# yewzijian/RegTR

Hardware: AMD Instinct MI355X
Metric: point-cloud pairs/sec (3DMatch ~20k pts) (higher is better)
Workload: dtype f32 (f16-pair split, 22-bit operands)

## Files before the change

### include/regtr_hip.h

```cpp
#ifndef REGTR_HIP_H
#define REGTR_HIP_H

#include <stddef.h>

#ifdef __cplusplus
extern "C" {
#endif

#define REGTR_OK 0
#define REGTR_ERR_LAUNCH (-1)
#define REGTR_ERR_ARG (-2)
#define REGTR_ERR_WORKSPACE (-3)

#define REGTR_ABI_VERSION 11
int regtr_abi_version(void);

#define REGTR_STATUS_F16_RANGE 1
#define REGTR_STATUS_NONFINITE_POSE 2


size_t regtr_grid_subsample_ws_bytes(int n_cap, int n_clouds);

int regtr_grid_subsample(const float* xyz, const int* seg_off, int n_clouds, int n_cap, float dl, float* out_xyz,
                         int* out_seg_off, void* ws, size_t ws_bytes, void* stream);

size_t regtr_grid_subsample_ordered_ws_bytes(int n_cap, int n_clouds, int row_order);
int regtr_grid_subsample_ordered(const float* xyz, const int* seg_off, int n_clouds, int n_cap, float dl, int row_order, int key_mode,
                                 int out_cap, float* out_xyz, int* out_seg_off, void* ws, size_t ws_bytes, void* stream);

size_t regtr_cellgrid_ws_bytes(int ns_cap, int n_clouds);

int regtr_cellgrid_build(const float* s_xyz, const int* s_seg_off, int n_clouds, int ns_cap, float radius, void* ws,
                         size_t ws_bytes, void* stream);

int regtr_radius_query(const float* q_xyz, const int* q_seg_off, int nq_cap, const int* s_seg_off, int ns_cap,
                       int n_clouds, float radius, int K, int order, const void* grid_ws, size_t ws_bytes, int* out_idx,
                       int* out_count, int* out_max_count, void* stream);

int regtr_radius_query_self(const int* s_seg_off, int ns_cap, int n_clouds, float radius, int K, int order, const void* grid_ws,
                            size_t ws_bytes, int* out_idx, int* out_count, int* out_max_count, void* stream);


int regtr_nearest_in_radius(const float* q_xyz, const int* q_seg_off, int nq_cap, const int* s_seg_off, int ns_cap,
                            int n_clouds, double radius, float grid_radius, const void* grid_ws, size_t ws_bytes, int* out_idx,
                            void* stream);

int regtr_overlap_avgpool(const float* ov, int ns, const int* nbr, int ld_nbr, int nq, int H, float* out, void* stream);



int regtr_rowsum_positive(const float* x, int n, int C, const float* stats, const int* seg_off, int n_seg, float slope,
                          float* flag, void* stream);

int regtr_kpconv_gather_computes_flag(int Cin, int H);

int regtr_kpconv_gather(const float* q_xyz, int nq, const float* s_xyz, int ns, const int* nbr, int H, const float* x,
                        int Cin, const float* flag, const float* s_xyzf, const float* kernel_points, int KP, float extent,
                        const float* x_stats, const int* q_seg_off, int n_seg, float slope, float* wf, int ld_wf, float* num,
                        void* stream);

int regtr_maxpool_gather(const float* x, int ns, int C, const int* nbr, int ld_nbr, int nq, int H, float* out, void* stream);

size_t regtr_instnorm_ws_bytes(int n_clouds, int max_len, int C);
int regtr_instnorm_stats(const float* x, const int* seg_off, int n_clouds, int max_len, int C, float eps, float* stats,
                         void* ws, size_t ws_bytes, void* stream);
int regtr_instnorm_apply(const float* x, const int* seg_off, int n_clouds, int max_len, int C, const float* stats,
                         const float* residual, const float* res_stats, int act, float slope, float* y, const float* row_xyz,
                         float* row_positive, void* stream);


size_t regtr_gemm_f32_ws_bytes(int M, int N, int K);
int regtr_gemm_f32(const float* A, int lda, const float* B, int ldb, float* C, int ldc, int M, int N, int K,
                   const float* bias, const float* row_div, const float* residual, int ldr, int act,
                   const float* a_stats, const int* a_seg_off, int n_seg, float a_slope, void* ws, size_t ws_bytes,
                   void* stream);

int regtr_gemm_x3_supported(int M, int N, int K);
int regtr_gemm_x3_preferred(int M, int N, int K);
size_t regtr_gemm_split_weights_bytes(int N, int K);
int regtr_gemm_split_weights(const float* W, int ld, int N, int K, int transposed, void* planes, void* stream);
int regtr_gemm_x3_f16_supported(int M, int N, int K, int with_stats);
size_t regtr_gemm_split_weights_f16_bytes(int N, int K);
int regtr_gemm_split_weights_f16(const float* W, int ld, int N, int K, int transposed, void* planes, void* stream);
size_t regtr_gemm_x3_ws_bytes(int M, int N, int K);
int regtr_gemm_x3(const float* A, int lda, const void* planes, float* C, int ldc, int M, int N, int K,
                  const float* bias, const float* row_div, const float* residual, int ldr, int act,
                  const float* a_stats, const int* a_seg_off, int n_seg, float a_slope, void* ws, size_t ws_bytes,
                  double* stat_partial, const int* stat_seg_off, int n_stat_seg, int n_planes, const void* tile_info, int* status,
                  void* stream);
int regtr_tile_segments(const int* seg_off, int n_seg, int M, int rows, void* out, void* stream);
int regtr_gemm_x3_tile_rows(int M, int N, int K);
int regtr_gemm_stream_supported(int M, int N, int K);
int regtr_gemm_stream_tile_rows(void);
int regtr_gemm_stream(const float* A, int lda, const void* planes, float* C, int ldc, int M, int N, int K,
                      const float* a_stats, float a_slope, const int* seg_off, int n_seg, const void* tile_info,
                      double* stat_partial, void* stream);
int regtr_block_tail_supported(int M, int N, int K1, int K2);
size_t regtr_block_tail_ws_bytes(int n_clouds, int max_len, int N, int K1, int K2);
int regtr_block_tail(const float* A1, int lda1, const float* a1_stats, float a1_slope, const float* row_div1, const float* A2, int lda2,
                     const float* W1, const float* W2, const int* seg_off, int n_clouds, int max_len, const void* tile_info,
                     int M, int N, int K1, int K2, float eps, float slope, float* Y, int ldy, void* ws, size_t ws_bytes,
                     float* out_stats, void* stream);

int regtr_gemm_x3_stat_tile_rows(int M, int N, int K);
int regtr_instnorm_finalize_tiles(const double* partial, const int* seg_off, int n_clouds, int C, int tile_rows, float eps,
                                  float* stats, void* stream);

int regtr_add_f32(const float* a, const float* b, size_t n, float* out, void* stream);

int regtr_layernorm(const float* x, int n, int D, const float* gamma, const float* beta, float eps, const float* add,
                    float* y, float* y_plain, void* stream);

int regtr_posemb_sine(const float* xyz, int n, int npf, int d_model, float scale, const float* dim_t, float* pe,
                      void* stream);


int regtr_mha_fwd(const float* q, int ldq, const float* k, int ldk, const float* v, int ldv, float* out, int ldo,
                  const int* seg_off, const int* kv_of, int n_clouds, int max_len, int n_heads, int head_dim, float scale,
                  int precision, int* status, void* stream);

int regtr_cross_encoder_per_layer_params(void);
int regtr_cross_encoder_supported(int n_tok, int d_model, int d_ff, int n_heads);
size_t regtr_cross_encoder_ws_bytes(int n_tok, int d_model, int d_ff);
int regtr_cross_encoder_fwd(const float* x, int n_tok, int d_model, int d_ff, int n_heads, int n_layers,
                            const void* const* layer_params, const float* layer_eps, const float* final_gamma,
                            const float* final_beta, float final_eps, int return_intermediate, const float* pe,
                            const int* seg_off, const int* kv_self, const int* kv_cross, int n_clouds, int max_len,
                            int gemm_planes, int attn_precision, void* ws, size_t ws_bytes, float* outs, int* status, void* stream);

typedef struct {
    const float* kn;
    const void* planes;
    const void* planes16;
    int N, K;
} regtr_weight_t;
typedef struct {
    int kind;
    int strided;
    int layer;
    int n_kp;
    float extent;
    const float* kernel_points;
    regtr_weight_t unary1;
    regtr_weight_t conv;
    regtr_weight_t unary2;
    regtr_weight_t shortcut;
} regtr_encoder_block_t;
typedef struct {
    const float* points;
    int n;
    const int* conv_idx;
    const int* pool_idx;
    int K;
    int pool_width;
    const int* seg_off;
    int max_len;
} regtr_encoder_level_t;
int regtr_encoder_supported(const regtr_encoder_block_t* blocks, int n_blocks, const regtr_encoder_level_t* levels, int n_levels,
                            int n_clouds, int first, int last);
size_t regtr_encoder_ws_bytes(const regtr_encoder_block_t* blocks, int n_blocks, const regtr_encoder_level_t* levels, int n_levels,
                              int n_clouds, int first, int last, int f16_pair);
int regtr_encoder_fwd(const regtr_encoder_block_t* blocks, int n_blocks, const regtr_encoder_level_t* levels, int n_levels, int n_clouds,
                      int first, int last, const float* x_in, float* out, int f16_pair, float slope, float eps, void* ws, size_t ws_bytes,
                      int* status, void* stream);

int regtr_attn_xyz(const float* q, const float* k, const float* xyz, float* out, const int* seg_off, const int* kv_of,
                   int n_clouds, int n_total, int n_layers, int max_len, int head_dim, float scale, void* stream);

int regtr_weighted_procrustes(const float* kp, const float* corr, const float* logit, const int* seg_off, int n_pairs,
                              int n_total, int n_layers, float* pose, int* status, void* stream);



size_t regtr_infonce_ws_bytes(int n_pairs, int max_anc);
int regtr_infonce(const float* anc, int ld_anc, const float* pos, int ld_pos, const float* anc_xyz, const float* pos_xyz,
                  const int* anc_seg_off, const int* pos_seg_off, int n_pairs, int n_anc, int n_pos, int max_anc, int D,
                  float r_p, float r_n, const float* anc_pose, float* pair_out, float* row_loss, float* row_mask, void* ws,
                  size_t ws_bytes, void* stream);

int regtr_se3_transform(const float* xyz, const int* seg_off, int n_clouds, int n, const float* pose, int pose_stride, float* out,
                        void* stream);

int regtr_loss_terms(const float* logit, const float* gt_overlap, const float* kp, const float* warped, const int* seg_off,
                     int n_pairs, int n_total, const float* pose, int pose_stride, float* out, void* stream);



int regtr_infonce_rows(const float* anc, int ld_anc, const float* pos, int ld_pos, const float* anc_xyz, const float* pos_xyz,
                       const int* anc_seg_off, const int* pos_seg_off, int n_pairs, int n_anc, int n_pos, int max_anc, int D,
                       float r_p, float r_n, const float* anc_pose, float* pair_out, float* row_loss, float* row_mask, float* row_lse,
                       int* row_idx, void* ws, size_t ws_bytes, void* stream);

int regtr_infonce_bwd(const float* anc, int ld_anc, const float* pos, int ld_pos, const float* anc_xyz, const float* pos_xyz,
                      const int* anc_seg_off, const int* pos_seg_off, int n_pairs, int n_anc, int n_pos, int max_anc, int max_pos,
                      int D, float r_n, const float* anc_pose, const float* row_lse, const int* row_idx, const float* row_mask,
                      const float* pair_out, const float* grad, float mean_div, float* d_anc, int ld_danc, float* d_pos, int ld_dpos,
                      void* stream);

size_t regtr_gemm_tn_ws_bytes(int M, int N1, int N2);
int regtr_gemm_tn(const float* a, int lda, const float* b, int ldb, int M, int N1, int N2, int fold, float* out, int ldo, void* ws,
                  size_t ws_bytes, void* stream);

int regtr_corr_l1_bwd(const float* kp, const float* warped, const float* w, const int* seg_off, int n_clouds, int n, const float* pose,
                      int pose_stride, const float* grad, const float* den, float* d_warped, void* stream);

size_t regtr_mha_bwd_ws_bytes(int n_total, int n_heads);
int regtr_mha_bwd(const float* q, int ldq, const float* k, int ldk, const float* v, int ldv, const float* d_out, int ld_do,
                  float* dq, int ld_dq, float* dk, int ld_dk, float* dv, int ld_dv, const int* seg_off, const int* kv_of,
                  int n_clouds, int n_total, int max_len, int n_heads, int head_dim, float scale, void* ws, size_t ws_bytes,
                  void* stream);

size_t regtr_layernorm_bwd_ws_bytes(int n, int D);
int regtr_layernorm_bwd(const float* x, int n, int D, const float* gamma, float eps, const float* dy, const float* dres, float* dx,
                        float* dgamma, float* dbeta, void* ws, size_t ws_bytes, void* stream);

size_t regtr_bias_relu_bwd_ws_bytes(int n, int N);
int regtr_bias_relu_bwd(const float* g, int ldg, const float* h, int ldh, float* dh, int ld_dh, float* db, int n, int N, void* ws,
                        size_t ws_bytes, void* stream);


size_t regtr_nbr_transpose_ws_bytes(int nq, int H, int ns);
int regtr_nbr_transpose(const int* nbr, int nq, int H, int ns, int* row_off, int* entries, void* ws, size_t ws_bytes, void* stream);

int regtr_kpconv_gather_bwd(const float* dwf, const float* q_xyz, int nq, const float* s_xyz, int ns, int H, int Cin,
                            const float* kernel_points, int KP, float extent, const int* row_off, const int* entries, float* dx,
                            void* stream);

int regtr_row_div(const float* x, int ldx, const float* div, int n, int N, float* out, int ldo, void* stream);

size_t regtr_gemm_tn_any_ws_bytes(int M, int N1, int N2);
int regtr_gemm_tn_any(const float* a, int lda, const float* b, int ldb, int M, int N1, int N2, float* out, int ldo, void* ws,
                      size_t ws_bytes, void* stream);

#ifdef __cplusplus
}
#endif
#endif
```

### regtr_amd/_lib.py

```python
import ctypes
import os
import threading

import torch

from . import context

_HERE = os.path.dirname(os.path.abspath(__file__))
LIB_PATH = os.path.join(_HERE, 'libregtr_hip.so')
if os.environ.get('REGTR_DEV', '') == '1' and os.environ.get('REGTR_VARIANT'):
    LIB_PATH = os.path.join(_HERE, f"libregtr_hip.{os.environ['REGTR_VARIANT']}.so")

_c = ctypes
_P = _c.c_void_p
_I = _c.c_int
_F = _c.c_float
_Z = _c.c_size_t

class Weight(_c.Structure):
    _fields_ = [('kn', _P), ('planes', _P), ('planes16', _P), ('N', _I), ('K', _I)]


class EncoderBlock(_c.Structure):
    _fields_ = [('kind', _I), ('strided', _I), ('layer', _I), ('n_kp', _I), ('extent', _F), ('kernel_points', _P),
                ('unary1', Weight), ('conv', Weight), ('unary2', Weight), ('shortcut', Weight)]


class EncoderLevel(_c.Structure):
    _fields_ = [('points', _P), ('n', _I), ('conv_idx', _P), ('pool_idx', _P), ('K', _I), ('pool_width', _I), ('seg_off', _P), ('max_len', _I)]


ABI_VERSION = 11

PARITY_SIGNATURES = {
    'regtr_parity_abi_version': (_I, []),
    'regtr_kdtree_ws_bytes': (_Z, [_I, _I]),
    'regtr_kdtree_query_scratch_bytes': (_Z, [_I]),
    'regtr_kdtree_build': (_I, [_P, _P, _I, _I, _P, _Z, _P]),
    'regtr_kdtree_radius_query': (_I, [_P, _P, _I, _P, _P, _I, _I, _F, _I, _I, _P, _Z, _P, _Z, _P, _P, _P, _P, _P]),
}

SIGNATURES = {
    'regtr_abi_version': (_I, []),
    'regtr_grid_subsample_ws_bytes': (_Z, [_I, _I]),
    'regtr_grid_subsample': (_I, [_P, _P, _I, _I, _F, _P, _P, _P, _Z, _P]),
    'regtr_grid_subsample_ordered_ws_bytes': (_Z, [_I, _I, _I]),
    'regtr_grid_subsample_ordered': (_I, [_P, _P, _I, _I, _F, _I, _I, _I, _P, _P, _P, _Z, _P]),
    'regtr_cellgrid_ws_bytes': (_Z, [_I, _I]),
    'regtr_cellgrid_build': (_I, [_P, _P, _I, _I, _F, _P, _Z, _P]),
    'regtr_radius_query': (_I, [_P, _P, _I, _P, _I, _I, _F, _I, _I, _P, _Z, _P, _P, _P, _P]),
    'regtr_radius_query_self': (_I, [_P, _I, _I, _F, _I, _I, _P, _Z, _P, _P, _P, _P]),
    'regtr_nearest_in_radius': (_I, [_P, _P, _I, _P, _I, _I, _c.c_double, _F, _P, _Z, _P, _P]),
    'regtr_overlap_avgpool': (_I, [_P, _I, _P, _I, _I, _I, _P, _P]),
    'regtr_rowsum_positive': (_I, [_P, _I, _I, _P, _P, _I, _F, _P, _P]),
    'regtr_kpconv_gather_computes_flag': (_I, [_I, _I]),
    'regtr_kpconv_gather': (_I, [_P, _I, _P, _I, _P, _I, _P, _I, _P, _P, _P, _I, _F, _P, _P, _I, _F, _P, _I, _P, _P]),
    'regtr_maxpool_gather': (_I, [_P, _I, _I, _P, _I, _I, _I, _P, _P]),
    'regtr_instnorm_ws_bytes': (_Z, [_I, _I, _I]),
    'regtr_instnorm_stats': (_I, [_P, _P, _I, _I, _I, _F, _P, _P, _Z, _P]),
    'regtr_instnorm_apply': (_I, [_P, _P, _I, _I, _I, _P, _P, _P, _I, _F, _P, _P, _P, _P]),
    'regtr_gemm_f32_ws_bytes': (_Z, [_I, _I, _I]),
    'regtr_gemm_f32': (_I, [_P, _I, _P, _I, _P, _I, _I, _I, _I, _P, _P, _P, _I, _I, _P, _P, _I, _F, _P, _Z, _P]),
    'regtr_gemm_x3_supported': (_I, [_I, _I, _I]),
    'regtr_gemm_x3_preferred': (_I, [_I, _I, _I]),
    'regtr_gemm_split_weights_bytes': (_Z, [_I, _I]),
    'regtr_gemm_split_weights': (_I, [_P, _I, _I, _I, _I, _P, _P]),
    'regtr_gemm_x3_f16_supported': (_I, [_I, _I, _I, _I]),
    'regtr_gemm_split_weights_f16_bytes': (_Z, [_I, _I]),
    'regtr_gemm_split_weights_f16': (_I, [_P, _I, _I, _I, _I, _P, _P]),
    'regtr_gemm_x3_ws_bytes': (_Z, [_I, _I, _I]),
    'regtr_gemm_x3': (_I, [_P, _I, _P, _P, _I, _I, _I, _I, _P, _P, _P, _I, _I, _P, _P, _I, _F, _P, _Z, _P, _P, _I, _I, _P, _P, _P]),
    'regtr_tile_segments': (_I, [_P, _I, _I, _I, _P, _P]),
    'regtr_gemm_x3_tile_rows': (_I, [_I, _I, _I]),
    'regtr_gemm_stream_supported': (_I, [_I, _I, _I]),
    'regtr_gemm_stream_tile_rows': (_I, []),
    'regtr_block_tail_supported': (_I, [_I, _I, _I, _I]),
    'regtr_block_tail_ws_bytes': (_Z, [_I, _I, _I, _I, _I]),
    'regtr_block_tail': (_I, [_P, _I, _P, _F, _P, _P, _I, _P, _P, _P, _I, _I, _P, _I, _I, _I, _I, _F, _F, _P, _I, _P, _Z, _P, _P]),
    'regtr_gemm_stream': (_I, [_P, _I, _P, _P, _I, _I, _I, _I, _P, _F, _P, _I, _P, _P, _P]),
    'regtr_gemm_x3_stat_tile_rows': (_I, [_I, _I, _I]),
    'regtr_instnorm_finalize_tiles': (_I, [_P, _P, _I, _I, _I, _F, _P, _P]),
    'regtr_add_f32': (_I, [_P, _P, _Z, _P, _P]),
    'regtr_layernorm': (_I, [_P, _I, _I, _P, _P, _F, _P, _P, _P, _P]),
    'regtr_posemb_sine': (_I, [_P, _I, _I, _I, _F, _P, _P, _P]),
    'regtr_mha_fwd': (_I, [_P, _I, _P, _I, _P, _I, _P, _I, _P, _P, _I, _I, _I, _I, _F, _I, _P, _P]),
    'regtr_cross_encoder_per_layer_params': (_I, []),
    'regtr_cross_encoder_supported': (_I, [_I, _I, _I, _I]),
    'regtr_cross_encoder_ws_bytes': (_Z, [_I, _I, _I]),
    'regtr_cross_encoder_fwd': (_I, [_P, _I, _I, _I, _I, _I, _P, _P, _P, _P, _F, _I, _P, _P, _P, _P, _I, _I, _I, _I, _P, _Z, _P, _P, _P]),
    'regtr_encoder_supported': (_I, [_P, _I, _P, _I, _I, _I, _I]),
    'regtr_encoder_ws_bytes': (_Z, [_P, _I, _P, _I, _I, _I, _I, _I]),
    'regtr_encoder_fwd': (_I, [_P, _I, _P, _I, _I, _I, _I, _P, _P, _I, _F, _F, _P, _Z, _P, _P]),
    'regtr_attn_xyz': (_I, [_P, _P, _P, _P, _P, _P, _I, _I, _I, _I, _I, _F, _P]),
    'regtr_weighted_procrustes': (_I, [_P, _P, _P, _P, _I, _I, _I, _P, _P, _P]),
    'regtr_infonce_ws_bytes': (_Z, [_I, _I]),
    'regtr_infonce': (_I, [_P, _I, _P, _I, _P, _P, _P, _P, _I, _I, _I, _I, _I, _F, _F, _P, _P, _P, _P, _P, _Z, _P]),
    'regtr_loss_terms': (_I, [_P, _P, _P, _P, _P, _I, _I, _P, _I, _P, _P]),
    'regtr_se3_transform': (_I, [_P, _P, _I, _I, _P, _I, _P, _P]),
    'regtr_infonce_rows': (_I, [_P, _I, _P, _I, _P, _P, _P, _P, _I, _I, _I, _I, _I, _F, _F, _P, _P, _P, _P, _P, _P, _P, _Z, _P]),
    'regtr_infonce_bwd': (_I, [_P, _I, _P, _I, _P, _P, _P, _P, _I, _I, _I, _I, _I, _I, _F, _P, _P, _P, _P, _P, _P, _F, _P, _I, _P, _I,
                               _P]),
    'regtr_gemm_tn_ws_bytes': (_Z, [_I, _I, _I]),
    'regtr_gemm_tn': (_I, [_P, _I, _P, _I, _I, _I, _I, _I, _P, _I, _P, _Z, _P]),
    'regtr_corr_l1_bwd': (_I, [_P, _P, _P, _P, _I, _I, _P, _I, _P, _P, _P, _P]),
    'regtr_mha_bwd_ws_bytes': (_Z, [_I, _I]),
    'regtr_mha_bwd': (_I, [_P, _I, _P, _I, _P, _I, _P, _I, _P, _I, _P, _I, _P, _I, _P, _P, _I, _I, _I, _I, _I, _F, _P, _Z, _P]),
    'regtr_layernorm_bwd_ws_bytes': (_Z, [_I, _I]),
    'regtr_layernorm_bwd': (_I, [_P, _I, _I, _P, _F, _P, _P, _P, _P, _P, _P, _Z, _P]),
    'regtr_bias_relu_bwd_ws_bytes': (_Z, [_I, _I]),
    'regtr_bias_relu_bwd': (_I, [_P, _I, _P, _I, _P, _I, _P, _I, _I, _P, _Z, _P]),
    'regtr_nbr_transpose_ws_bytes': (_Z, [_I, _I, _I]),
    'regtr_nbr_transpose': (_I, [_P, _I, _I, _I, _P, _P, _P, _Z, _P]),
    'regtr_kpconv_gather_bwd': (_I, [_P, _P, _I, _P, _I, _I, _I, _P, _I, _F, _P, _P, _P, _P]),
    'regtr_row_div': (_I, [_P, _I, _P, _I, _I, _P, _I, _P]),
    'regtr_gemm_tn_any_ws_bytes': (_Z, [_I, _I, _I]),
    'regtr_gemm_tn_any': (_I, [_P, _I, _P, _I, _I, _I, _I, _P, _I, _P, _Z, _P]),
}

COMPOSITE = ('regtr_encoder_fwd', 'regtr_cross_encoder_fwd')

_ERR = {-1: 'kernel launch failed', -2: 'invalid argument', -3: 'workspace too small'}

_lib = None
_load_lock = threading.Lock()


def lib():
    global _lib
    if _lib is None:
        with _load_lock:
            if _lib is None:
                _lib = _load()
    return _lib


def _load():
    _lib = None
    if True:
        if not os.path.exists(LIB_PATH):
            raise RuntimeError(f'{LIB_PATH} is missing: build it with `python -m regtr_amd.build` '
                               '(hipcc --offload-arch=gfx950). There is no CPU fallback.')
        _lib = ctypes.PyDLL(LIB_PATH)
        for name, (res, args) in SIGNATURES.items():
            fn = getattr(_lib, name)
            fn.restype = res
            fn.argtypes = args
        nogil = ctypes.CDLL(LIB_PATH)
        for name in COMPOSITE:
            fn = getattr(nogil, name)
            fn.restype, fn.argtypes = SIGNATURES[name]
            setattr(_lib, name, fn)
        got = _lib.regtr_abi_version()
        if got != ABI_VERSION:
            _lib = None
            raise RuntimeError(f'{LIB_PATH} implements C-ABI version {got}, this binding was written for {ABI_VERSION}: rebuild with '
                               '`python -m regtr_amd.build --force`')
    return _lib


_parity = None
PARITY_LIB_PATH = os.path.join(_HERE, 'libregtr_parity.so')


def parity_lib():
    global _parity
    if _parity is None:
        with _load_lock:
            if _parity is None:
                if not os.path.exists(PARITY_LIB_PATH):
                    raise RuntimeError(f'{PARITY_LIB_PATH} is missing: build it with `python -m regtr_amd.build` (parity mode only)')
                lib_ = ctypes.PyDLL(PARITY_LIB_PATH)
                for name, (res, args) in PARITY_SIGNATURES.items():
                    fn = getattr(lib_, name)
                    fn.restype, fn.argtypes = res, args
                if lib_.regtr_parity_abi_version() != ABI_VERSION:
                    raise RuntimeError(f'{PARITY_LIB_PATH} was built against C-ABI version {lib_.regtr_parity_abi_version()}, this binding is {ABI_VERSION}: '
                                       'rebuild with `python -m regtr_amd.build --force`')
                _parity = lib_
    return _parity


def check(status, what):
    if status != 0:
        raise RuntimeError(f'{what}: {_ERR.get(status, "error")} (status {status})')


on_device = context.on_device


def ptr(t, dtype=torch.float32):
    if t is None:
        return None
    dev = context.current().device_index
    if t.get_device() != (dev if dev is not None else torch.cuda.current_device()) or t.dtype is not dtype or not t.is_contiguous():
        _explain(t, dtype)
    return t.data_ptr()


def _explain(t, dtype):
    if not t.is_cuda:
        raise RuntimeError('regtr_amd ops need GPU tensors (no CPU fallback)')
    if t.dtype != dtype:
        raise RuntimeError(f'regtr_amd op expected a {dtype} tensor, got {t.dtype} (the kernels reinterpret nothing)')
    if not t.is_contiguous():
        raise RuntimeError('regtr_amd ops need contiguous tensors')
    dev = context.current().device_index
    raise RuntimeError(f'tensor on {t.device} but the launch device is cuda:{dev if dev is not None else torch.cuda.current_device()}; '
                       'wrap the call in regtr_amd._lib.on_device(tensor.device)')


def iptr(t):
    return ptr(t, torch.int32)


def bptr(t):
    return ptr(t, torch.uint8)


def dptr(t):
    return ptr(t, torch.float64)


def raw(t):
    if t is None:
        return None
    if t.dtype is not torch.float32 or t.get_device() < 0:
        raise RuntimeError(f'regtr_amd op expected a float32 GPU tensor, got {t.dtype} on {t.device}')
    return t.data_ptr()


_raw_stream = getattr(torch._C, '_cuda_getCurrentRawStream', None)


def stream():
    dev = context.current().device_index
    if _raw_stream is not None:
        return _raw_stream(dev if dev is not None else torch.cuda.current_device())
    return torch.cuda.current_stream().cuda_stream
```

### regtr_amd/csrc/attention.hip

```cpp
#include "common.h"
#include "mfma_operands.h"

namespace {

constexpr int HD = 32;
constexpr int TQ = 32, TK = 32;
constexpr int LDS_STRIDE = HD + 1;

struct MhaArgs {
    const float* q; const float* k; const float* v;
    float* out;
    const int* seg_off; const int* kv_of;
    int ldq, ldk, ldv, ldo, n_heads;
    float scale;
    int* status;
};

__device__ __forceinline__ int acc_row(int r, int hi) { return (r & 3) + 8 * (r >> 2) + 4 * hi; }

template <int KS>
__global__ void __launch_bounds__(KS * RG_WAVE) __attribute__((amdgpu_waves_per_eu(2))) k_mha_fwd(MhaArgs g)
{
    __shared__ float KVs[KS][2 * TK * LDS_STRIDE];
    const int lane = threadIdx.x & 63, l31 = lane & 31, hi = lane >> 5;
    const int wave = __builtin_amdgcn_readfirstlane(threadIdx.x >> 6);
    float* Ks = KVs[wave];
    float* Vs = KVs[wave] + TK * LDS_STRIDE;
    const int cloud = blockIdx.z, head = blockIdx.y;
    const int q_begin = g.seg_off[cloud], q_end = g.seg_off[cloud + 1];
    const int q0 = q_begin + blockIdx.x * TQ;
    if (q0 >= q_end) return;
    const int kc = g.kv_of[cloud];
    const int k_begin = g.seg_off[kc], nk = g.seg_off[kc + 1] - k_begin;
    const int hoff = head * HD;

    float qreg[16];
    {
        const int qrow = q0 + l31;
        const bool live = qrow < q_end;
        const float* qp = g.q + (size_t)(live ? qrow : q_begin) * g.ldq + hoff + hi;
        const float scl = live ? g.scale : 0.f;
#pragma unroll
        for (int s = 0; s < 16; s++) qreg[s] = qp[2 * s] * scl;
    }

    floatx16 o;
#pragma unroll
    for (int r = 0; r < 16; r++) o[r] = 0.f;
    float m_run = -INFINITY, l_run = 0.f;

    float4 kreg[4], vreg[4];
    auto fetch = [&](int kt) {
#pragma unroll
        for (int it = 0; it < 4; it++) {
            const int krow = min(kt + it * 8 + (lane >> 3), nk > 0 ? nk - 1 : 0), c4 = (lane & 7) * 4;
            const int kb = nk > 0 ? k_begin : q_begin;
            kreg[it] = *(const float4*)(g.k + (size_t)(kb + krow) * g.ldk + hoff + c4);
            vreg[it] = *(const float4*)(g.v + (size_t)(kb + krow) * g.ldv + hoff + c4);
        }
    };
    fetch(wave * TK);
    for (int kt = wave * TK; kt < nk; kt += KS * TK) {
        __builtin_amdgcn_wave_barrier();
#pragma unroll
        for (int it = 0; it < 4; it++) {
            const int row = it * 8 + (lane >> 3), c4 = (lane & 7) * 4;
            float* kd = &Ks[row * LDS_STRIDE + c4];
            kd[0] = kreg[it].x; kd[1] = kreg[it].y; kd[2] = kreg[it].z; kd[3] = kreg[it].w;
            float* vd = &Vs[row * LDS_STRIDE + c4];
            vd[0] = vreg[it].x; vd[1] = vreg[it].y; vd[2] = vreg[it].z; vd[3] = vreg[it].w;
        }
        __builtin_amdgcn_wave_barrier();
        fetch(kt + KS * TK);

        floatx16 sc;
#pragma unroll
        for (int r = 0; r < 16; r++) sc[r] = 0.f;
#pragma unroll
        for (int s = 0; s < 16; s++)
            sc = __builtin_amdgcn_mfma_f32_32x32x2f32(Ks[l31 * LDS_STRIDE + 2 * s + hi], qreg[s], sc, 0, 0, 0);

        float mx = -INFINITY;
#pragma unroll
        for (int r = 0; r < 16; r++) {
            if (kt + acc_row(r, hi) >= nk) sc[r] = -INFINITY;
            mx = fmaxf(mx, sc[r]);
        }
        mx = fmaxf(mx, __shfl_xor(mx, 32, RG_WAVE));
        const float m_new = fmaxf(m_run, mx);
        const float alpha = expf(m_run - m_new);
        float psum = 0.f;
#pragma unroll
        for (int r = 0; r < 16; r++) {
            sc[r] = expf(sc[r] - m_new);
            psum += sc[r];
        }
        psum += __shfl_xor(psum, 32, RG_WAVE);
        l_run = l_run * alpha + psum;
        m_run = m_new;
#pragma unroll
        for (int r = 0; r < 16; r++) o[r] *= alpha;

#pragma unroll
        for (int s = 0; s < 16; s++)
            o = __builtin_amdgcn_mfma_f32_32x32x2f32(Vs[acc_row(s, hi) * LDS_STRIDE + l31], sc[s], o, 0, 0, 0);
    }

    if (KS > 1) {
        __builtin_amdgcn_wave_barrier();
        float* mine = KVs[wave];
        if (wave > 0) {
#pragma unroll
            for (int r = 0; r < 16; r++) mine[r * 64 + lane] = o[r];
            mine[16 * 64 + lane] = m_run;
            mine[17 * 64 + lane] = l_run;
        }
        __syncthreads();
        if (wave > 0) return;
#pragma unroll 1
        for (int w = 1; w < KS; w++) {
            const float* p = KVs[w];
            const float mw = p[16 * 64 + lane], lw = p[17 * 64 + lane];
            if (mw == -INFINITY) continue;
            const float m_new = fmaxf(m_run, mw);
            const float a0 = expf(m_run - m_new), a1 = expf(mw - m_new);
            l_run = l_run * a0 + lw * a1;
#pragma unroll
            for (int r = 0; r < 16; r++) o[r] = o[r] * a0 + p[r * 64 + lane] * a1;
            m_run = m_new;
        }
    }

    const int qrow = q0 + l31;
    if (qrow < q_end) {
        const float inv = l_run > 0.f ? 1.0f / l_run : 0.f;
        float* dst = g.out + (size_t)qrow * g.ldo + hoff;
#pragma unroll
        for (int r4 = 0; r4 < 4; r4++) {
            const int d = 8 * r4 + 4 * hi;
            *(float4*)(dst + d) = make_float4(o[4 * r4] * inv, o[4 * r4 + 1] * inv, o[4 * r4 + 2] * inv, o[4 * r4 + 3] * inv);
        }
    }
}

constexpr int BW = 4;
constexpr int BW8 = 8;
constexpr int BROW = 64;

#ifndef MHA_WAVES_ATTR
#define MHA_WAVES_ATTR __attribute__((amdgpu_waves_per_eu(3)))
#endif
#ifndef MHA_WIDE_MIN_WG
#define MHA_WIDE_MIN_WG 4096
#endif
template <int NP, bool F16 = false>
__device__ __forceinline__ void bf_split8(const float (&x)[8], bf16x8 (&f)[NP])
{
    unsigned w[4][NP];
#pragma unroll
    for (int i = 0; i < 4; i++) rg_split2<NP, F16>(x[2 * i], x[2 * i + 1], w[i]);
#pragma unroll
    for (int p = 0; p < NP; p++) f[p] = __builtin_bit_cast(bf16x8, make_uint4(w[0][p], w[1][p], w[2][p], w[3][p]));
}
template <int NP>
__device__ __forceinline__ floatx16 bf_mma(const bf16x8 (&a)[NP], const bf16x8 (&b)[NP], floatx16 c)
{
    if (NP == 3) {
        c = __builtin_amdgcn_mfma_f32_32x32x16_bf16(a[2], b[0], c, 0, 0, 0);
        c = __builtin_amdgcn_mfma_f32_32x32x16_bf16(a[1], b[1], c, 0, 0, 0);
        c = __builtin_amdgcn_mfma_f32_32x32x16_bf16(a[0], b[2], c, 0, 0, 0);
    }
    if (NP >= 2) {
        c = __builtin_amdgcn_mfma_f32_32x32x16_bf16(a[1], b[0], c, 0, 0, 0);
        c = __builtin_amdgcn_mfma_f32_32x32x16_bf16(a[0], b[1], c, 0, 0, 0);
    }
    return __builtin_amdgcn_mfma_f32_32x32x16_bf16(a[0], b[0], c, 0, 0, 0);
}

__device__ __forceinline__ void f16_mma(const bf16x8 (&a)[2], const bf16x8 (&b)[2], floatx16& hi, floatx16& lo)
{
    lo = __builtin_amdgcn_mfma_f32_32x32x16_f16(__builtin_bit_cast(f16x8, a[1]), __builtin_bit_cast(f16x8, b[0]), lo, 0, 0, 0);
    hi = __builtin_amdgcn_mfma_f32_32x32x16_f16(__builtin_bit_cast(f16x8, a[0]), __builtin_bit_cast(f16x8, b[0]), hi, 0, 0, 0);
    lo = __builtin_amdgcn_mfma_f32_32x32x16_f16(__builtin_bit_cast(f16x8, a[0]), __builtin_bit_cast(f16x8, b[1]), lo, 0, 0, 0);
}

__device__ __forceinline__ float mha_max_halves(float x)
{
    const auto r = __builtin_amdgcn_permlane32_swap(__float_as_uint(x), __float_as_uint(x), false, false);
    return fmaxf(__uint_as_float(r[0]), __uint_as_float(r[1]));
}
__device__ __forceinline__ float mha_sum_halves(float x)
{
    const auto r = __builtin_amdgcn_permlane32_swap(__float_as_uint(x), __float_as_uint(x), false, false);
    return __uint_as_float(r[0]) + __uint_as_float(r[1]);
}

template <int NP, bool F16 = false, int NW = BW>
__global__ void __launch_bounds__(NW * RG_WAVE) MHA_WAVES_ATTR k_mha_fwd_bf16(MhaArgs g)
{
    __shared__ __align__(16) unsigned char Ks[2][NP][TK * BROW];
    __shared__ __align__(16) unsigned char Vt[2][NP][HD * BROW];
    const int t = threadIdx.x, lane = t & 63, l31 = lane & 31, hi = lane >> 5;
    const int wave = __builtin_amdgcn_readfirstlane(t >> 6);
    const int cloud = blockIdx.z, head = blockIdx.y;
    const int q_begin = g.seg_off[cloud], q_end = g.seg_off[cloud + 1];
    if (q_begin + (int)blockIdx.x * NW * TQ >= q_end) return;
    const int q0 = q_begin + (blockIdx.x * NW + wave) * TQ;
    const bool wave_live = q0 < q_end;
    const int kc = g.kv_of[cloud];
    const int k_begin = g.seg_off[kc], nk = g.seg_off[kc + 1] - k_begin;
    const int hoff = head * HD;

    bf16x8 qf[2][NP];
    {
        const int qrow = q0 + l31;
        const bool live = wave_live && qrow < q_end;
        const float sc2 = g.scale * 1.44269504088896340736f;
        const float* qp = g.q + (size_t)(live ? qrow : q_begin) * g.ldq + hoff + 8 * hi;
        float4 qv[2][2];
#pragma unroll
        for (int ks = 0; ks < 2; ks++) { qv[ks][0] = *(const float4*)(qp + 16 * ks); qv[ks][1] = *(const float4*)(qp + 16 * ks + 4); }
        const float scl = live ? sc2 : 0.f;
#pragma unroll
        for (int ks = 0; ks < 2; ks++) {
            const float x[8] = {qv[ks][0].x * scl, qv[ks][0].y * scl, qv[ks][0].z * scl, qv[ks][0].w * scl,
                                qv[ks][1].x * scl, qv[ks][1].y * scl, qv[ks][1].z * scl, qv[ks][1].w * scl};
            bf_split8<NP, F16>(x, qf[ks]);
        }
    }

    constexpr int KPT = NW == 4 ? 4 : 2;
    const int skey = t / (32 / KPT), sdk = (t % (32 / KPT)) * KPT;
    const int su = NW == 4 ? t >> 4 : t >> 5, sd2 = NW == 4 ? (t & 15) * 2 : (t & 31);
    const unsigned k_dst = (unsigned)skey * BROW + (((unsigned)(sdk >> 3) ^ (((unsigned)skey >> 2) & 3u)) * 16u) + ((unsigned)sdk & 7u) * 2u;
    const unsigned vpos = ((2u * su) & 0x13u) | (((2u * su) & 4u) << 1) | (((2u * su) & 8u) >> 1);
    unsigned v_dst[2];
#pragma unroll
    for (int dd = 0; dd < 2; dd++) {
        const unsigned row = (unsigned)(sd2 + dd);
        v_dst[dd] = row * BROW + (((vpos >> 3) ^ ((row >> 2) & 3u)) * 16u) + (vpos & 7u) * 2u;
    }
    struct KV { float4 k; float2 v0, v1; };
    const int nk1 = nk > 0 ? nk - 1 : 0;
    const int kb = nk > 0 ? k_begin : q_begin;
    auto fetch = [&](KV& r, int kt) {
        const int kr = min(kt + skey, nk1), v0 = min(kt + 2 * su, nk1), v1 = min(kt + 2 * su + 1, nk1);
        if constexpr (NW == 4) {
            r.k = *(const float4*)(g.k + (size_t)(kb + kr) * g.ldk + hoff + sdk);
            r.v0 = *(const float2*)(g.v + (size_t)(kb + v0) * g.ldv + hoff + sd2);
            r.v1 = *(const float2*)(g.v + (size_t)(kb + v1) * g.ldv + hoff + sd2);
        } else {
            const float2 k2 = *(const float2*)(g.k + (size_t)(kb + kr) * g.ldk + hoff + sdk);
            r.k.x = k2.x; r.k.y = k2.y;
            r.v0.x = g.v[(size_t)(kb + v0) * g.ldv + hoff + sd2];
            r.v1.x = g.v[(size_t)(kb + v1) * g.ldv + hoff + sd2];
        }
    };
    auto stage = [&](const KV& r, int buf) {
        unsigned a[NP], b[NP];
        rg_split2<NP, F16>(r.k.x, r.k.y, a);
        if constexpr (NW == 4) {
            rg_split2<NP, F16>(r.k.z, r.k.w, b);
#pragma unroll
            for (int p = 0; p < NP; p++) *(uint2*)(&Ks[buf][p][k_dst]) = make_uint2(a[p], b[p]);
        } else {
#pragma unroll
            for (int p = 0; p < NP; p++) *(unsigned*)(&Ks[buf][p][k_dst]) = a[p];
        }
        rg_split2<NP, F16>(r.v0.x, r.v1.x, a);
        if constexpr (NW == 4) rg_split2<NP, F16>(r.v0.y, r.v1.y, b);
#pragma unroll
        for (int p = 0; p < NP; p++) {
            *(unsigned*)(&Vt[buf][p][v_dst[0]]) = a[p];
            if constexpr (NW == 4) *(unsigned*)(&Vt[buf][p][v_dst[1]]) = b[p];
        }
    };

    floatx16 o, o_lo;
#pragma unroll
    for (int r = 0; r < 16; r++) { o[r] = 0.f; o_lo[r] = 0.f; }
    float m_run = -INFINITY, l_run = 0.f;
    unsigned f_off[2];
#pragma unroll
    for (int ks = 0; ks < 2; ks++) f_off[ks] = (unsigned)l31 * BROW + ((((unsigned)(2 * ks + hi)) ^ (((unsigned)l31 >> 2) & 3u)) * 16u);

#ifdef MHA_PROF
    long long pt[6] = {0, 0, 0, 0, 0, 0}, pc = clock64(), pstart = pc;
#define MHA_STAMP(I) do { const long long n_ = clock64(); pt[I] += n_ - pc; pc = n_; } while (0)
#else
#define MHA_STAMP(I) do {} while (0)
#endif
    KV ra, rb;
    fetch(ra, 0);
    stage(ra, 0);
    fetch(ra, TK);
    __syncthreads();
    MHA_STAMP(0);
    auto tile = [&](int kt, int buf, KV& rold, KV& rnew) {
        const bool more = kt + TK < nk;
        fetch(rnew, kt + 2 * TK);
        MHA_STAMP(1);
        if (wave_live) {
            floatx16 sc, sc_lo;
#pragma unroll
            for (int r = 0; r < 16; r++) { sc[r] = 0.f; sc_lo[r] = 0.f; }
#pragma unroll
            for (int ks = 0; ks < 2; ks++) {
                bf16x8 kf[NP];
#pragma unroll
                for (int p = 0; p < NP; p++) kf[p] = __builtin_bit_cast(bf16x8, *(const uint4*)(&Ks[buf][p][f_off[ks]]));
                if constexpr (F16) f16_mma(kf, qf[ks], sc, sc_lo);
                else sc = bf_mma<NP>(kf, qf[ks], sc);
            }
            if constexpr (F16) {
                rg_fold_low(sc, sc_lo);
            }
            MHA_STAMP(2);
            if (kt + TK > nk) {
#pragma unroll
                for (int r = 0; r < 16; r++)
                    if (kt + acc_row(r, hi) >= nk) sc[r] = -INFINITY;
            }
            float mx = -INFINITY;
#pragma unroll
            for (int r = 0; r < 16; r++) mx = fmaxf(mx, sc[r]);
            mx = mha_max_halves(mx);
            const float m_new = fmaxf(m_run, mx);
            const float alpha = __builtin_amdgcn_exp2f(m_run - m_new);
            float pr[16];
            float psum = 0.f;
#pragma unroll
            for (int r = 0; r < 16; r++) { pr[r] = __builtin_amdgcn_exp2f(sc[r] - m_new); psum += pr[r]; }
            psum = mha_sum_halves(psum);
            l_run = l_run * alpha + psum;
            m_run = m_new;
#pragma unroll
            for (int r = 0; r < 16; r++) { o[r] *= alpha; if (F16) o_lo[r] *= alpha; }
#pragma unroll
            for (int ks = 0; ks < 2; ks++) {
                float x[8];
#pragma unroll
                for (int j = 0; j < 8; j++) x[j] = pr[8 * ks + j];
                bf16x8 pf[NP], vf[NP];
                bf_split8<NP, F16>(x, pf);
#pragma unroll
                for (int p = 0; p < NP; p++) vf[p] = __builtin_bit_cast(bf16x8, *(const uint4*)(&Vt[buf][p][f_off[ks]]));
                if constexpr (F16) f16_mma(vf, pf, o, o_lo);
                else o = bf_mma<NP>(vf, pf, o);
            }
            MHA_STAMP(3);
        }
        if (more) stage(rold, buf ^ 1);
        MHA_STAMP(4);
        __syncthreads();
        MHA_STAMP(5);
    };
    for (int kt = 0; kt < nk; kt += 2 * TK) {
        tile(kt, 0, ra, rb);
        if (kt + TK >= nk) break;
        tile(kt + TK, 1, rb, ra);
    }
#ifdef MHA_PROF
    if ((blockIdx.z == 3 || blockIdx.z == 77) && blockIdx.y == 2 && lane == 0)
        printf("mha NP %d cloud %d wg %d wave %d live %d nk %d: prologue %lld fetch-issue %lld qk %lld softmax+pv %lld stage %lld barrier %lld total %lld (cycles)\n", NP,
               (int)blockIdx.z, (int)blockIdx.x, wave, (int)wave_live, nk, pt[0], pt[1], pt[2], pt[3], pt[4], pt[5], clock64() - pstart);
#endif

    if constexpr (F16) {
        const float chk = fmaf(l_run, 0.f, rg_fold_low(o, o_lo));
        rg_report_range(g.status, chk, wave_live);
    }
    const int qrow = q0 + l31;
    if (wave_live && qrow < q_end) {
        const float inv = l_run > 0.f ? 1.0f / l_run : 0.f;
        float* dst = g.out + (size_t)qrow * g.ldo + hoff;
#pragma unroll
        for (int r4 = 0; r4 < 4; r4++) {
            const int d = 8 * r4 + 4 * hi;
            *(float4*)(dst + d) = make_float4(o[4 * r4] * inv, o[4 * r4 + 1] * inv, o[4 * r4 + 2] * inv, o[4 * r4 + 3] * inv);
        }
    }
}

struct AttnXyzArgs {
    const float* q; const float* k; const float* xyz; float* out;
    const int* seg_off; const int* kv_of;
    int n_total;
    float scale;
};

template <int HDX>
__global__ void __launch_bounds__(RG_WAVE) __attribute__((amdgpu_waves_per_eu(2))) k_attn_xyz(AttnXyzArgs g)
{
    constexpr int KS = HDX + 1;
    extern __shared__ float smem_x[];
    float* Ks = smem_x;
    float* Vs = smem_x + TK * KS;
    const int lane = threadIdx.x, l31 = lane & 31, hi = lane >> 5;
    const int cloud = blockIdx.z, layer = blockIdx.y;
    const int q_begin = g.seg_off[cloud], q_end = g.seg_off[cloud + 1];
    const int q0 = q_begin + blockIdx.x * TQ;
    if (q0 >= q_end) return;
    const int kc = g.kv_of[cloud];
    const int k_begin = g.seg_off[kc], nk = g.seg_off[kc + 1] - k_begin;
    const float* Q = g.q + (size_t)layer * g.n_total * HDX;
    const float* K = g.k + (size_t)layer * g.n_total * HDX;

    float qreg[HDX / 2];
    {
        const int qrow = q0 + l31;
        const bool live = qrow < q_end;
        const float* qp = Q + (size_t)(live ? qrow : q_begin) * HDX + hi;
        const float scl = live ? g.scale : 0.f;
#pragma unroll
        for (int s = 0; s < HDX / 2; s++) qreg[s] = qp[2 * s] * scl;
    }
    floatx16 o;
#pragma unroll
    for (int r = 0; r < 16; r++) o[r] = 0.f;
    float m_run = -INFINITY, l_run = 0.f;
    for (int e = lane; e < TK * LDS_STRIDE; e += RG_WAVE) Vs[e] = 0.f;

    constexpr int LPR = HDX / 4 < RG_WAVE ? HDX / 4 : RG_WAVE;
    const int c4 = (lane < LPR ? lane : LPR - 1) * 4;
    const int nk1 = nk > 0 ? nk - 1 : 0;
    const int kb = nk > 0 ? k_begin : q_begin;
    for (int kt = 0; kt < nk; kt += TK) {
        __syncthreads();
#pragma unroll 1
        for (int row0 = 0; row0 < TK; row0 += 8) {
            float4 v[8];
#pragma unroll
            for (int i = 0; i < 8; i++) v[i] = *(const float4*)(K + (size_t)(kb + min(kt + row0 + i, nk1)) * HDX + c4);
            if (lane < LPR) {
#pragma unroll
                for (int i = 0; i < 8; i++) {
                    float* kd = &Ks[(row0 + i) * KS + c4];
                    kd[0] = v[i].x; kd[1] = v[i].y; kd[2] = v[i].z; kd[3] = v[i].w;
                }
            }
        }
        {
            const float* xp = g.xyz + (size_t)(kb + min(kt + l31, nk1)) * 3;
            const float x = xp[0], y = xp[1], z = xp[2];
            if (hi == 0) { Vs[l31 * LDS_STRIDE] = x; Vs[l31 * LDS_STRIDE + 1] = y; Vs[l31 * LDS_STRIDE + 2] = z; }
        }
        __syncthreads();

        floatx16 sc;
#pragma unroll
        for (int r = 0; r < 16; r++) sc[r] = 0.f;
#pragma unroll
        for (int s = 0; s < HDX / 2; s++)
            sc = __builtin_amdgcn_mfma_f32_32x32x2f32(Ks[l31 * KS + 2 * s + hi], qreg[s], sc, 0, 0, 0);

        float mx = -INFINITY;
#pragma unroll
        for (int r = 0; r < 16; r++) {
            if (kt + acc_row(r, hi) >= nk) sc[r] = -INFINITY;
            mx = fmaxf(mx, sc[r]);
        }
        mx = fmaxf(mx, __shfl_xor(mx, 32, RG_WAVE));
        const float m_new = fmaxf(m_run, mx);
        const float alpha = expf(m_run - m_new);
        float psum = 0.f;
#pragma unroll
        for (int r = 0; r < 16; r++) {
            sc[r] = expf(sc[r] - m_new);
            psum += sc[r];
        }
        psum += __shfl_xor(psum, 32, RG_WAVE);
        l_run = l_run * alpha + psum;
        m_run = m_new;
#pragma unroll
        for (int r = 0; r < 16; r++) o[r] *= alpha;
#pragma unroll
        for (int s = 0; s < 16; s++)
            o = __builtin_amdgcn_mfma_f32_32x32x2f32(Vs[acc_row(s, hi) * LDS_STRIDE + l31], sc[s], o, 0, 0, 0);
    }
    const int qrow = q0 + l31;
    if (qrow < q_end && hi == 0) {
        const float inv = l_run > 0.f ? 1.0f / l_run : 0.f;
        float* dst = g.out + ((size_t)layer * g.n_total + qrow) * 3;
        dst[0] = o[0] * inv; dst[1] = o[1] * inv; dst[2] = o[2] * inv;
    }
}

}

extern "C" {

int regtr_mha_fwd(const float* q, int ldq, const float* k, int ldk, const float* v, int ldv, float* out, int ldo,
                  const int* seg_off, const int* kv_of, int n_clouds, int max_len, int n_heads, int head_dim, float scale,
                  int precision, int* status, void* stream)
{
    if (!q || !k || !v || !out || !seg_off || !kv_of || n_clouds < 1 || n_heads < 1 || max_len < 0) return RG_ERR_ARG;
    if (head_dim != HD || precision < 0 || precision > 3) return RG_ERR_ARG;
    if ((ldq | ldk | ldv | ldo) % 4 || (((uintptr_t)q | (uintptr_t)k | (uintptr_t)v | (uintptr_t)out) % 16)) return RG_ERR_ARG;
    if (max_len == 0) return RG_OK;
    MhaArgs g{q, k, v, out, seg_off, kv_of, ldq, ldk, ldv, ldo, n_heads, scale, status};
    hipStream_t st = (hipStream_t)stream;
    const bool small = (long long)rg_cdiv(max_len, BW * TQ) * n_heads * n_clouds < 512;
    if (precision == 2 || ((precision == 0 || precision == 3) && small)) {
        const dim3 grid(rg_cdiv(max_len, TQ), n_heads, n_clouds);
        if ((long long)grid.x * grid.y * grid.z <= 1024 && max_len > 4 * TK) k_mha_fwd<4><<<grid, 4 * RG_WAVE, 0, st>>>(g);
        else k_mha_fwd<1><<<grid, RG_WAVE, 0, st>>>(g);
    }
    else {
        if ((ldv % 2) || ((uintptr_t)v % 8)) return RG_ERR_ARG;
        if (max_len > BW * TQ && (long long)rg_cdiv(max_len, BW8 * TQ) * n_heads * n_clouds >= MHA_WIDE_MIN_WG) {
            const dim3 grid(rg_cdiv(max_len, BW8 * TQ), n_heads, n_clouds);
            if (precision == 0) k_mha_fwd_bf16<3, false, BW8><<<grid, BW8 * RG_WAVE, 0, st>>>(g);
            else if (precision == 3) k_mha_fwd_bf16<2, true, BW8><<<grid, BW8 * RG_WAVE, 0, st>>>(g);
            else k_mha_fwd_bf16<1, false, BW8><<<grid, BW8 * RG_WAVE, 0, st>>>(g);
        } else {
            const dim3 grid(rg_cdiv(max_len, BW * TQ), n_heads, n_clouds);
            if (precision == 0) k_mha_fwd_bf16<3><<<grid, BW * RG_WAVE, 0, st>>>(g);
            else if (precision == 3) k_mha_fwd_bf16<2, true><<<grid, BW * RG_WAVE, 0, st>>>(g);
            else k_mha_fwd_bf16<1><<<grid, BW * RG_WAVE, 0, st>>>(g);
        }
    }
    RG_RETURN_IF_LAUNCH_FAILED();
    return RG_OK;
}

int regtr_attn_xyz(const float* q, const float* k, const float* xyz, float* out, const int* seg_off, const int* kv_of,
                   int n_clouds, int n_total, int n_layers, int max_len, int head_dim, float scale, void* stream)
{
    if (!q || !k || !xyz || !out || !seg_off || !kv_of || n_clouds < 1 || n_total < 0 || n_layers < 1 || max_len < 0)
        return RG_ERR_ARG;
    if ((((uintptr_t)q | (uintptr_t)k) % 16)) return RG_ERR_ARG;
    if (max_len == 0 || n_total == 0) return RG_OK;
    AttnXyzArgs g{q, k, xyz, out, seg_off, kv_of, n_total, scale};
    const dim3 grid(rg_cdiv(max_len, TQ), n_layers, n_clouds);
    hipStream_t st = (hipStream_t)stream;
#define RG_ATTN_XYZ(HDX_) k_attn_xyz<HDX_><<<grid, RG_WAVE, (TK * (HDX_ + 1) + TK * LDS_STRIDE) * sizeof(float), st>>>(g)
    if (head_dim == 256) RG_ATTN_XYZ(256);
    else if (head_dim == 128) RG_ATTN_XYZ(128);
    else if (head_dim == 64) RG_ATTN_XYZ(64);
    else if (head_dim == 32) RG_ATTN_XYZ(32);
    else return RG_ERR_ARG;
#undef RG_ATTN_XYZ
    RG_RETURN_IF_LAUNCH_FAILED();
    return RG_OK;
}

}
```

### regtr_amd/csrc/cross_encoder.hip

```cpp
#include <math.h>

#include "common.h"

namespace {

enum {
    CE_N1_G, CE_N1_B, CE_SA_IN_W, CE_SA_IN_B, CE_SA_OUT_W, CE_SA_OUT_B,
    CE_N2_G, CE_N2_B, CE_CA_IN_W, CE_CA_IN_B, CE_CA_OUT_W, CE_CA_OUT_B,
    CE_N3_G, CE_N3_B, CE_L1_W, CE_L1_B, CE_L2_W, CE_L2_B, CE_PER_LAYER
};

size_t ce_gemm_ws(int M, int D, int F)
{
    size_t w = regtr_gemm_x3_ws_bytes(M, 3 * D, D);
    const size_t a = regtr_gemm_x3_ws_bytes(M, D, D), b = regtr_gemm_x3_ws_bytes(M, F, D), c = regtr_gemm_x3_ws_bytes(M, D, F);
    if (a > w) w = a;
    if (b > w) w = b;
    if (c > w) w = c;
    return w;
}

}

extern "C" {

int regtr_cross_encoder_per_layer_params(void) { return CE_PER_LAYER; }

int regtr_cross_encoder_supported(int n_tok, int d_model, int d_ff, int n_heads)
{
    if (n_tok < 1 || d_model < 64 || d_ff < 64 || n_heads < 1 || d_model % n_heads || d_model / n_heads != 32) return 0;
    return (regtr_gemm_x3_preferred(n_tok, 3 * d_model, d_model) && regtr_gemm_x3_preferred(n_tok, d_model, d_model) &&
            regtr_gemm_x3_preferred(n_tok, d_ff, d_model) && regtr_gemm_x3_preferred(n_tok, d_model, d_ff)) ? 1 : 0;
}

size_t regtr_cross_encoder_ws_bytes(int n_tok, int d_model, int d_ff)
{
    const size_t row = (size_t)n_tok * sizeof(float);
    return 6 * 256 + row * ((size_t)d_model * 4 + 3 * (size_t)d_model + d_ff) + rg_align_up(ce_gemm_ws(n_tok, d_model, d_ff), 256) + 256;
}

int regtr_cross_encoder_fwd(const float* x, int n_tok, int d_model, int d_ff, int n_heads, int n_layers,
                            const void* const* layer_params, const float* layer_eps, const float* final_gamma,
                            const float* final_beta, float final_eps, int return_intermediate, const float* pe,
                            const int* seg_off, const int* kv_self, const int* kv_cross, int n_clouds, int max_len,
                            int gemm_planes, int attn_precision, void* ws, size_t ws_bytes, float* outs, int* status, void* stream)
{
    if (!x || !layer_params || !layer_eps || !seg_off || !kv_self || !kv_cross || !outs || n_layers < 1 || n_clouds < 1) return RG_ERR_ARG;
    if (!regtr_cross_encoder_supported(n_tok, d_model, d_ff, n_heads)) return RG_ERR_ARG;
    if (!ws || ws_bytes < regtr_cross_encoder_ws_bytes(n_tok, d_model, d_ff)) return RG_ERR_WORKSPACE;
    const int M = n_tok, D = d_model, F = d_ff, hd = D / n_heads;
    RgCarver cv(ws, ws_bytes);
    float* x2p = cv.take<float>((size_t)M * D);
    float* qkv = cv.take<float>((size_t)M * 3 * D);
    float* att = cv.take<float>((size_t)M * D);
    float* xa = cv.take<float>((size_t)M * D);
    float* xb = cv.take<float>((size_t)M * D);
    float* h = cv.take<float>((size_t)M * F);
    const size_t gws_bytes = ce_gemm_ws(M, D, F);
    void* gws = gws_bytes ? (void*)cv.take<char>(gws_bytes) : nullptr;
    if (!cv.ok()) return RG_ERR_WORKSPACE;
    const float scale = (float)(1.0 / sqrt((double)hd));

#define CE_TRY(call) do { const int st_ = (call); if (st_ != RG_OK) return st_; } while (0)
    auto gemm = [&](const float* A, int K, const void* W, const void* bias, float* C, int N, const float* residual, int relu) {
        return regtr_gemm_x3(A, K, W, C, N, M, N, K, (const float*)bias, nullptr, residual, residual ? D : 0, relu, nullptr, nullptr, 0,
                             0.1f, gws, gws_bytes, nullptr, nullptr, 0, gemm_planes, nullptr, status, stream);
    };
    auto attention = [&](const float* xin, const void* const* P, int g, int in_w, float eps, const int* kv_of, float* xout) {
        int st = regtr_layernorm(xin, M, D, (const float*)P[g], (const float*)P[g + 1], eps, pe, x2p, nullptr, stream);
        if (st != RG_OK) return st;
        st = gemm(x2p, D, P[in_w], P[in_w + 1], qkv, 3 * D, nullptr, 0);
        if (st != RG_OK) return st;
        st = regtr_mha_fwd(qkv, 3 * D, qkv + D, 3 * D, qkv + 2 * D, 3 * D, att, D, seg_off, kv_of, n_clouds, max_len, n_heads, hd, scale,
                           attn_precision, status, stream);
        if (st != RG_OK) return st;
        return gemm(att, D, P[in_w + 2], P[in_w + 3], xout, D, xin, 0);
    };

    const float* cur = x;
    for (int l = 0; l < n_layers; l++) {
        const void* const* P = layer_params + (size_t)l * CE_PER_LAYER;
        const float* eps = layer_eps + 3 * l;
        float* t1 = (cur == xa) ? xb : xa;
        float* t2 = (t1 == xa) ? xb : xa;
        CE_TRY(attention(cur, P, CE_N1_G, CE_SA_IN_W, eps[0], kv_self, t1));
        CE_TRY(attention(t1, P, CE_N2_G, CE_CA_IN_W, eps[1], kv_cross, t2));
        CE_TRY(regtr_layernorm(t2, M, D, (const float*)P[CE_N3_G], (const float*)P[CE_N3_B], eps[2], nullptr, x2p, nullptr, stream));
        CE_TRY(gemm(x2p, D, P[CE_L1_W], P[CE_L1_B], h, F, nullptr, 1));
        CE_TRY(gemm(h, F, P[CE_L2_W], P[CE_L2_B], t1, D, t2, 0));
        cur = t1;
        if (return_intermediate || l == n_layers - 1) {
            float* o = outs + (return_intermediate ? (size_t)l * M * D : 0);
            if (final_gamma) CE_TRY(regtr_layernorm(cur, M, D, final_gamma, final_beta, final_eps, nullptr, o, nullptr, stream));
            else if (hipMemcpyAsync(o, cur, (size_t)M * D * sizeof(float), hipMemcpyDeviceToDevice, (hipStream_t)stream) != hipSuccess)
                return RG_ERR_LAUNCH;
        }
    }
#undef CE_TRY
    return RG_OK;
}

}
```

### regtr_amd/csrc/norm.hip

```cpp
#include "common.h"

namespace {

constexpr int IN_ROWS = 128;

inline int in_rows(int max_len, int n_clouds, int C)
{
    const int TR = 256 / (C >> 2);
    int rows = IN_ROWS;
    while (rows > 4 * TR && rows > 8 && (long long)rg_cdiv(max_len > 0 ? max_len : 1, rows) * n_clouds < 1024) rows >>= 1;
    return rows;
}


__global__ void __launch_bounds__(256) k_instnorm_partial(const float* __restrict__ x, const int* __restrict__ seg_off, int C,
                                                          int nchunk, int rows, double2* __restrict__ partial)
{
    __shared__ double sh[256 * 8];
    const int b = blockIdx.y, chunk = blockIdx.x;
    const int r0 = seg_off[b] + chunk * rows, r1 = min(seg_off[b + 1], r0 + rows);
    if (r0 >= r1) return;
    const int C4 = C >> 2, TR = 256 / C4;
    const int tx = threadIdx.x % C4, ty = threadIdx.x / C4;
    double s[4] = {0, 0, 0, 0}, ss[4] = {0, 0, 0, 0};
    const float* base = x + 4 * tx;
    auto add = [&](const float4& v) {
        s[0] += v.x; s[1] += v.y; s[2] += v.z; s[3] += v.w;
        ss[0] += (double)v.x * v.x; ss[1] += (double)v.y * v.y; ss[2] += (double)v.z * v.z; ss[3] += (double)v.w * v.w;
    };
    int r = r0 + ty;
    for (; r + 3 * TR < r1; r += 4 * TR) {
        float4 v[4];
#pragma unroll
        for (int u = 0; u < 4; u++) v[u] = *(const float4*)(base + (size_t)(r + u * TR) * C);
#pragma unroll
        for (int u = 0; u < 4; u++) add(v[u]);
    }
    for (; r < r1; r += TR) add(*(const float4*)(base + (size_t)r * C));
#pragma unroll
    for (int j = 0; j < 4; j++) { sh[threadIdx.x * 8 + j] = s[j]; sh[threadIdx.x * 8 + 4 + j] = ss[j]; }
    __syncthreads();
    if (ty == 0) {
        for (int y = 1; y < TR; y++)
#pragma unroll
            for (int j = 0; j < 4; j++) { s[j] += sh[(y * C4 + tx) * 8 + j]; ss[j] += sh[(y * C4 + tx) * 8 + 4 + j]; }
        double2* o = partial + ((size_t)b * nchunk + chunk) * C + 4 * tx;
#pragma unroll
        for (int j = 0; j < 4; j++) o[j] = make_double2(s[j], ss[j]);
    }
}

__global__ void __launch_bounds__(256) k_instnorm_finalize(const double2* __restrict__ partial, const int* __restrict__ seg_off,
                                                           int C, int nchunk, int rows, float eps, float2* __restrict__ stats)
{
    const int b = blockIdx.y, c = blockIdx.x * (blockDim.x >> 6) + (threadIdx.x >> 6);
    if (c >= C) return;
    const int lane = rg_lane();
    const int n = seg_off[b + 1] - seg_off[b];
    const int used = (n + rows - 1) / rows;
    double s = 0, ss = 0;
    for (int k = lane; k < used; k += RG_WAVE) {
        const double2 p = partial[((size_t)b * nchunk + k) * C + c];
        s += p.x; ss += p.y;
    }
    s = rg_wave_sum(s); ss = rg_wave_sum(ss);
    if (lane == 0) {
        float mean = 0.f, rstd = 0.f;
        if (n > 0) {
            const double m = s / n;
            double var = ss / n - m * m;
            if (var < 0) var = 0;
            mean = (float)m;
            rstd = (float)(1.0 / sqrt(var + (double)eps));
        }
        stats[(size_t)b * C + c] = make_float2(mean, rstd);
    }
}

__global__ void __launch_bounds__(256) k_instnorm_finalize_tiles(const double2* __restrict__ partial, const int* __restrict__ seg_off,
                                                                 int C, int tile_rows, float eps, float2* __restrict__ stats)
{
    const int b = blockIdx.y, c = blockIdx.x * blockDim.x + threadIdx.x;
    if (c >= C) return;
    const int r0 = seg_off[b], r1 = seg_off[b + 1], n = r1 - r0;
    float mean = 0.f, rstd = 0.f;
    if (n > 0) {
        const int t0 = r0 / tile_rows, t1 = (r1 - 1) / tile_rows;
        const double2* p = partial + (size_t)(t0 + b) * C + c;
        double s = 0, ss = 0;
        int t = t0;
        for (; t + 3 <= t1; t += 4) {
            const double2 a0 = p[0], a1 = p[(size_t)C], a2 = p[2 * (size_t)C], a3 = p[3 * (size_t)C];
            s = (((s + a0.x) + a1.x) + a2.x) + a3.x; ss = (((ss + a0.y) + a1.y) + a2.y) + a3.y;
            p += 4 * (size_t)C;
        }
        for (; t <= t1; t++) { const double2 a = *p; s += a.x; ss += a.y; p += C; }
        const double m = s / n;
        double var = ss / n - m * m;
        if (var < 0) var = 0;
        mean = (float)m;
        rstd = (float)(1.0 / sqrt(var + (double)eps));
    }
    stats[(size_t)b * C + c] = make_float2(mean, rstd);
}

__global__ void __launch_bounds__(256) k_instnorm_finalize_tiles_wave(const double2* __restrict__ partial, const int* __restrict__ seg_off,
                                                                      int C, int tile_rows, float eps, float2* __restrict__ stats)
{
    const int b = blockIdx.y, c = blockIdx.x * (blockDim.x >> 6) + (threadIdx.x >> 6);
    if (c >= C) return;
    const int lane = rg_lane();
    const int r0 = seg_off[b], r1 = seg_off[b + 1], n = r1 - r0;
    float mean = 0.f, rstd = 0.f;
    if (n > 0) {
        const int t0 = r0 / tile_rows, t1 = (r1 - 1) / tile_rows;
        double s = 0, ss = 0;
        for (int t = t0 + lane; t <= t1; t += RG_WAVE) {
            const double2 a = partial[(size_t)(t + b) * C + c];
            s += a.x; ss += a.y;
        }
        s = rg_wave_sum(s); ss = rg_wave_sum(ss);
        const double m = s / n;
        double var = ss / n - m * m;
        if (var < 0) var = 0;
        mean = (float)m;
        rstd = (float)(1.0 / sqrt(var + (double)eps));
    }
    if (lane == 0) stats[(size_t)b * C + c] = make_float2(mean, rstd);
}

__global__ void __launch_bounds__(256) k_instnorm_apply(const float* __restrict__ x, const int* __restrict__ seg_off, int C,
                                                        const float2* __restrict__ stats, const float* __restrict__ res,
                                                        const float2* __restrict__ res_stats, int act, float slope,
                                                        float* __restrict__ y, const float* __restrict__ row_xyz,
                                                        float* __restrict__ row_positive, int rows)
{
    const int b = blockIdx.y, chunk = blockIdx.x;
    const int r0 = seg_off[b] + chunk * rows, r1 = min(seg_off[b + 1], r0 + rows);
    if (r0 >= r1) return;
    const int C4 = C >> 2, TR = 256 / C4;
    const int tx = threadIdx.x % C4, ty = threadIdx.x / C4;
    float mu[4] = {0.f, 0.f, 0.f, 0.f}, rs[4] = {1.f, 1.f, 1.f, 1.f}, rmu[4] = {0.f, 0.f, 0.f, 0.f}, rrs[4] = {1.f, 1.f, 1.f, 1.f};
    if (stats) {
        const float4* st = (const float4*)(stats + (size_t)b * C + 4 * tx);
        const float4 a = st[0], c = st[1];
        mu[0] = a.x; rs[0] = a.y; mu[1] = a.z; rs[1] = a.w; mu[2] = c.x; rs[2] = c.y; mu[3] = c.z; rs[3] = c.w;
    }
    if (res_stats) {
        const float4* st = (const float4*)(res_stats + (size_t)b * C + 4 * tx);
        const float4 a = st[0], c = st[1];
        rmu[0] = a.x; rrs[0] = a.y; rmu[1] = a.z; rrs[1] = a.w; rmu[2] = c.x; rrs[2] = c.y; rmu[3] = c.z; rrs[3] = c.w;
    }
    for (int r = r0 + ty; r < r1; r += 4 * TR) {
        float4 v[4], rv[4];
#pragma unroll
        for (int u = 0; u < 4; u++) v[u] = *(const float4*)(x + (size_t)min(r + u * TR, r1 - 1) * C + 4 * tx);
        if (res) {
#pragma unroll
            for (int u = 0; u < 4; u++) rv[u] = *(const float4*)(res + (size_t)min(r + u * TR, r1 - 1) * C + 4 * tx);
        }
#pragma unroll
        for (int u = 0; u < 4; u++) {
            const int rr = r + u * TR;
            if (rr >= r1) continue;
            float o[4] = {v[u].x, v[u].y, v[u].z, v[u].w};
#pragma unroll
            for (int j = 0; j < 4; j++) o[j] = (o[j] - mu[j]) * rs[j];
            if (res) {
                const float q[4] = {rv[u].x, rv[u].y, rv[u].z, rv[u].w};
#pragma unroll
                for (int j = 0; j < 4; j++) o[j] += (q[j] - rmu[j]) * rrs[j];
            }
            if (act == 1) {
#pragma unroll
                for (int j = 0; j < 4; j++) o[j] = o[j] > 0.f ? o[j] : o[j] * slope;
            }
            *(float4*)(y + (size_t)rr * C + 4 * tx) = make_float4(o[0], o[1], o[2], o[3]);
            if (row_positive) {
                float sum = (o[0] + o[1]) + (o[2] + o[3]);
                for (int m = 1; m < C4; m <<= 1) sum += __shfl_xor(sum, m, RG_WAVE);
                if (tx == 0) {
                    const float f = sum > 0.f ? 1.f : 0.f;
                    if (row_xyz) *(float4*)(row_positive + 4 * (size_t)rr) = make_float4(row_xyz[3 * (size_t)rr], row_xyz[3 * (size_t)rr + 1],
                                                                                         row_xyz[3 * (size_t)rr + 2], f);
                    else row_positive[rr] = f;
                }
            }
        }
    }
}

__global__ void __launch_bounds__(256) k_layernorm(const float* __restrict__ x, int n, int D, const float* __restrict__ gamma,
                                                   const float* __restrict__ beta, float eps, const float* __restrict__ add,
                                                   float* __restrict__ y, float* __restrict__ y_plain)
{
    const int row = blockIdx.x * (blockDim.x >> 6) + (threadIdx.x >> 6);
    if (row >= n) return;
    const int lane = rg_lane();
    const float* xr = x + (size_t)row * D;
    float s = 0.f;
    for (int c = lane * 4; c < D; c += RG_WAVE * 4) {
        const float4 v = *(const float4*)(xr + c);
        s += (v.x + v.y) + (v.z + v.w);
    }
    const float mean = rg_wave_sum(s) / (float)D;
    float ss = 0.f;
    for (int c = lane * 4; c < D; c += RG_WAVE * 4) {
        const float4 v = *(const float4*)(xr + c);
        const float a = v.x - mean, b = v.y - mean, cc = v.z - mean, d = v.w - mean;
        ss += (a * a + b * b) + (cc * cc + d * d);
    }
    const float rstd = 1.0f / sqrtf(rg_wave_sum(ss) / (float)D + eps);
    for (int c = lane * 4; c < D; c += RG_WAVE * 4) {
        const float4 v = *(const float4*)(xr + c);
        const float4 gm = *(const float4*)(gamma + c), bt = *(const float4*)(beta + c);
        float4 o = make_float4((v.x - mean) * rstd * gm.x + bt.x, (v.y - mean) * rstd * gm.y + bt.y,
                               (v.z - mean) * rstd * gm.z + bt.z, (v.w - mean) * rstd * gm.w + bt.w);
        if (y_plain) *(float4*)(y_plain + (size_t)row * D + c) = o;
        if (add) {
            const float4 a = *(const float4*)(add + (size_t)row * D + c);
            o.x += a.x; o.y += a.y; o.z += a.z; o.w += a.w;
        }
        *(float4*)(y + (size_t)row * D + c) = o;
    }
}

__global__ void __launch_bounds__(256) k_posemb_sine(const float* __restrict__ xyz, int n, int npf, int d_model, float scale,
                                                     const float* __restrict__ dim_t, float* __restrict__ pe)
{
    const size_t e = (size_t)blockIdx.x * blockDim.x + threadIdx.x;
    if (e >= (size_t)n * d_model) return;
    const int i = (int)(e / d_model), d = (int)(e % d_model);
    float v = 0.f;
    if (d < 3 * npf) {
        const int a = d / npf, f = d % npf;
        const float p = __fdiv_rn(__fmul_rn(xyz[3 * (size_t)i + a], scale), dim_t[f]);
        v = (f & 1) ? cosf(p) : sinf(p);
    }
    pe[e] = v;
}

}

extern "C" {

size_t regtr_instnorm_ws_bytes(int n_clouds, int max_len, int C)
{
    if (n_clouds < 1 || C < 4 || C % 4 || C > 1024 || 256 % (C / 4)) return 256;
    const size_t nchunk = (size_t)rg_cdiv(max_len > 0 ? max_len : 1, in_rows(max_len, n_clouds, C));
    return nchunk * n_clouds * C * sizeof(double2) + 256;
}

int regtr_instnorm_stats(const float* x, const int* seg_off, int n_clouds, int max_len, int C, float eps, float* stats,
                         void* ws, size_t ws_bytes, void* stream)
{
    if (!x || !seg_off || !stats || n_clouds < 1 || C < 4 || C % 4 || max_len < 0) return RG_ERR_ARG;
    if (C > 1024 || 256 % (C / 4)) return RG_ERR_ARG;
    if (ws_bytes < regtr_instnorm_ws_bytes(n_clouds, max_len, C)) return RG_ERR_WORKSPACE;
    if (max_len == 0) return RG_OK;
    hipStream_t st = (hipStream_t)stream;
    const int rows = in_rows(max_len, n_clouds, C);
    const int nchunk = rg_cdiv(max_len, rows);
    k_instnorm_partial<<<dim3(nchunk, n_clouds), 256, 0, st>>>(x, seg_off, C, nchunk, rows, (double2*)ws);
    k_instnorm_finalize<<<dim3(rg_cdiv(C, 4), n_clouds), 256, 0, st>>>((const double2*)ws, seg_off, C, nchunk, rows, eps,
                                                                         (float2*)stats);
    RG_RETURN_IF_LAUNCH_FAILED();
    return RG_OK;
}

int regtr_instnorm_finalize_tiles(const double* partial, const int* seg_off, int n_clouds, int C, int tile_rows, float eps,
                                  float* stats, void* stream)
{
    if (!partial || !seg_off || !stats || n_clouds < 1 || C < 1 || tile_rows < 1) return RG_ERR_ARG;
    if ((long long)n_clouds * C <= 4096) {
        k_instnorm_finalize_tiles_wave<<<dim3(rg_cdiv(C, 4), n_clouds), 256, 0, (hipStream_t)stream>>>(
            (const double2*)partial, seg_off, C, tile_rows, eps, (float2*)stats);
    } else {
        const int bs = C >= 256 ? 256 : (C >= 128 ? 128 : 64);
        k_instnorm_finalize_tiles<<<dim3(rg_cdiv(C, bs), n_clouds), bs, 0, (hipStream_t)stream>>>(
            (const double2*)partial, seg_off, C, tile_rows, eps, (float2*)stats);
    }
    RG_RETURN_IF_LAUNCH_FAILED();
    return RG_OK;
}

int regtr_instnorm_apply(const float* x, const int* seg_off, int n_clouds, int max_len, int C, const float* stats,
                         const float* residual, const float* res_stats, int act, float slope, float* y, const float* row_xyz,
                         float* row_positive, void* stream)
{
    if (!x || !seg_off || !y || n_clouds < 1 || C < 4 || C % 4 || max_len < 0) return RG_ERR_ARG;
    if (C > 1024 || 256 % (C / 4) || (row_positive && C > 256) || (row_xyz && (!row_positive || (uintptr_t)row_positive % 16)))
        return RG_ERR_ARG;
    if (max_len == 0) return RG_OK;
    const int rows = in_rows(max_len, n_clouds, C);
    k_instnorm_apply<<<dim3(rg_cdiv(max_len, rows), n_clouds), 256, 0, (hipStream_t)stream>>>(
        x, seg_off, C, (const float2*)stats, residual, (const float2*)res_stats, act, slope, y, row_xyz, row_positive, rows);
    RG_RETURN_IF_LAUNCH_FAILED();
    return RG_OK;
}

static __global__ void __launch_bounds__(256) k_add(const float* __restrict__ a, const float* __restrict__ b, size_t n, float* __restrict__ out)
{
    const size_t i = ((size_t)blockIdx.x * blockDim.x + threadIdx.x) * 4;
    if (i + 3 < n) {
        const float4 x = *(const float4*)(a + i), y = *(const float4*)(b + i);
        *(float4*)(out + i) = make_float4(x.x + y.x, x.y + y.y, x.z + y.z, x.w + y.w);
    } else {
        for (size_t j = i; j < n; j++) out[j] = a[j] + b[j];
    }
}

int regtr_add_f32(const float* a, const float* b, size_t n, float* out, void* stream)
{
    if (!a || !b || !out || (((uintptr_t)a | (uintptr_t)b | (uintptr_t)out) % 16)) return RG_ERR_ARG;
    if (n == 0) return RG_OK;
    k_add<<<rg_cdiv((long long)((n + 3) / 4), 256), 256, 0, (hipStream_t)stream>>>(a, b, n, out);
    RG_RETURN_IF_LAUNCH_FAILED();
    return RG_OK;
}

int regtr_layernorm(const float* x, int n, int D, const float* gamma, const float* beta, float eps, const float* add,
                    float* y, float* y_plain, void* stream)
{
    if (!x || !gamma || !beta || !y || n < 0 || D < 4 || D % 4) return RG_ERR_ARG;
    if (n == 0) return RG_OK;
    k_layernorm<<<rg_cdiv(n, 4), 256, 0, (hipStream_t)stream>>>(x, n, D, gamma, beta, eps, add, y, y_plain);
    RG_RETURN_IF_LAUNCH_FAILED();
    return RG_OK;
}

int regtr_posemb_sine(const float* xyz, int n, int npf, int d_model, float scale, const float* dim_t, float* pe,
                      void* stream)
{
    if (!xyz || !dim_t || !pe || n < 0 || npf < 1 || d_model < 3 * npf) return RG_ERR_ARG;
    if (n == 0) return RG_OK;
    k_posemb_sine<<<rg_cdiv((long long)n * d_model, 256), 256, 0, (hipStream_t)stream>>>(xyz, n, npf, d_model, scale,
                                                                                          dim_t, pe);
    RG_RETURN_IF_LAUNCH_FAILED();
    return RG_OK;
}

}
```

### regtr_amd/ops.py

```python
import math

import torch

from . import _lib, context
from ._lib import bptr, check, dptr, iptr, ptr, raw, stream


def _ws(nbytes, device):
    return torch.empty(int(nbytes), dtype=torch.uint8, device=device)


F16_OPERAND_LIMIT = 65504.0 / 2


VOXEL_KEY_MODES = {'origin': 0, 'floor': 1, 'floor_rcp': 2}


def grid_subsample(xyz, seg_off, n_cap, dl, row_order=0, key_mode=0, out_cap=None):
    L = _lib.lib()
    n_clouds = seg_off.numel() - 1
    out_cap = int(n_cap if out_cap is None else min(out_cap, n_cap))
    out = torch.empty((max(out_cap, 1), 3), dtype=torch.float32, device=xyz.device)
    out_off = torch.empty(n_clouds + 1, dtype=torch.int32, device=xyz.device)
    nb = L.regtr_grid_subsample_ordered_ws_bytes(n_cap, n_clouds, int(row_order))
    ws = _ws(nb, xyz.device)
    check(L.regtr_grid_subsample_ordered(ptr(xyz), iptr(seg_off), n_clouds, n_cap, float(dl), int(row_order), int(key_mode), out_cap, ptr(out),
                                         iptr(out_off), bptr(ws), nb, stream()), 'regtr_grid_subsample_ordered')
    return out, out_off


self_query_kernel = True
SELF_QUERY_MIN_POINTS = 262144


class CellGrid:

    def __init__(self, s_xyz, s_seg_off, ns_cap, radius):
        L = _lib.lib()
        self.n_clouds = s_seg_off.numel() - 1
        self.s_xyz, self.s_seg_off, self.ns_cap, self.radius = s_xyz, s_seg_off, int(ns_cap), float(radius)
        self.nbytes = L.regtr_cellgrid_ws_bytes(self.ns_cap, self.n_clouds)
        self.ws = _ws(self.nbytes, s_xyz.device)
        check(L.regtr_cellgrid_build(ptr(s_xyz), iptr(s_seg_off), self.n_clouds, self.ns_cap, self.radius, bptr(self.ws),
                                     self.nbytes, stream()), 'regtr_cellgrid_build')

    def query(self, q_xyz, q_seg_off, nq_cap, K, want_count=False, order=0):
        L = _lib.lib()
        idx = torch.empty((max(nq_cap, 1), K), dtype=torch.int32, device=q_xyz.device)
        cnt = mx = None
        if want_count:
            cnt = torch.empty(max(nq_cap, 1), dtype=torch.int32, device=q_xyz.device)
            mx = torch.zeros(1, dtype=torch.int32, device=q_xyz.device)
        if self_query_kernel and q_xyz is self.s_xyz and q_seg_off is self.s_seg_off and self.ns_cap >= SELF_QUERY_MIN_POINTS:
            check(L.regtr_radius_query_self(iptr(self.s_seg_off), self.ns_cap, self.n_clouds, self.radius, int(K), int(order),
                                            bptr(self.ws), self.nbytes, iptr(idx), iptr(cnt), iptr(mx), stream()), 'regtr_radius_query_self')
        else:
            check(L.regtr_radius_query(ptr(q_xyz), iptr(q_seg_off), int(nq_cap), iptr(self.s_seg_off), self.ns_cap,
                                       self.n_clouds, self.radius, int(K), int(order), bptr(self.ws), self.nbytes, iptr(idx), iptr(cnt),
                                       iptr(mx), stream()), 'regtr_radius_query')
        return (idx, cnt, mx) if want_count else idx


class KdTree:

    def __init__(self, s_xyz, s_seg_off, ns_cap):
        L = _lib.parity_lib()
        self.n_clouds = s_seg_off.numel() - 1
        self.s_xyz, self.s_seg_off, self.ns_cap = s_xyz, s_seg_off, int(ns_cap)
        self.nbytes = L.regtr_kdtree_ws_bytes(self.ns_cap, self.n_clouds)
        self.ws = _ws(self.nbytes, s_xyz.device)
        check(L.regtr_kdtree_build(ptr(s_xyz), iptr(s_seg_off), self.n_clouds, self.ns_cap, bptr(self.ws), self.nbytes, stream()),
              'regtr_kdtree_build')

    def query(self, q_xyz, q_seg_off, nq_cap, radius, K, list_cap=128):
        L = _lib.parity_lib()
        dev = q_xyz.device
        idx = torch.empty((max(nq_cap, 1), K), dtype=torch.int32, device=dev)
        while True:
            st = torch.zeros(2, dtype=torch.int32, device=dev)
            sb = L.regtr_kdtree_query_scratch_bytes(int(list_cap))
            scratch = _ws(sb, dev)
            check(L.regtr_kdtree_radius_query(ptr(q_xyz), iptr(q_seg_off), int(nq_cap), ptr(self.s_xyz), iptr(self.s_seg_off),
                                              self.ns_cap, self.n_clouds, float(radius), int(K), int(list_cap), bptr(self.ws),
                                              self.nbytes, bptr(scratch), sb, iptr(idx), None, st.data_ptr(), st.data_ptr() + 4,
                                              stream()), 'regtr_kdtree_radius_query')
            max_count, overflow = (int(v) for v in st.cpu())
            if overflow:
                raise RuntimeError('regtr_kdtree_radius_query: traversal stack overflow (tree deeper than the parity mode supports)')
            if max_count <= list_cap:
                break
            list_cap = max_count
        return idx, max_count


class SplitWeight:

    def __init__(self, w, layout):
        L = _lib.lib()
        w = w.detach().contiguous()
        if layout == 'nk':
            self.N, self.K = w.shape
            self.kn = w.t().contiguous()
        else:
            self.K, self.N = w.shape
            self.kn = w
        self.planes = None
        self._w, self._layout, self._planes16, self._f16_ok = w, layout, None, None
        if L.regtr_gemm_x3_supported(1, self.N, self.K) or L.regtr_gemm_stream_supported(1, self.N, self.K):
            self.planes = _ws(L.regtr_gemm_split_weights_bytes(self.N, self.K), w.device)
            check(L.regtr_gemm_split_weights(ptr(w), w.stride(0), self.N, self.K, 0 if layout == 'nk' else 1, bptr(self.planes),
                                             stream()), 'regtr_gemm_split_weights')


    @property
    def f16_ok(self):
        if self._f16_ok is None:
            self._f16_ok = bool(self._w.numel() == 0 or float(self._w.abs().max()) < F16_OPERAND_LIMIT)
        return self._f16_ok

    @property
    def planes16(self):
        if self._planes16 is None:
            L = _lib.lib()
            if not self.f16_ok:
                raise RuntimeError('SplitWeight.planes16: a weight of magnitude >= 65504 cannot take the f16 pair format (check .f16_ok)')
            self._planes16 = _ws(L.regtr_gemm_split_weights_f16_bytes(self.N, self.K), self._w.device)
            check(L.regtr_gemm_split_weights_f16(ptr(self._w), self._w.stride(0), self.N, self.K, 0 if self._layout == 'nk' else 1,
                                                 bptr(self._planes16), stream()), 'regtr_gemm_split_weights_f16')
        return self._planes16


_f16_shape = {}


def f16_pair(on):
    return context.current().derive(f16_pair=bool(on))


def f16_pair_ok(M, N, K, with_stats=False):
    key = (M, N, K, bool(with_stats))
    v = _f16_shape.get(key)
    if v is None:
        if len(_f16_shape) > 4096:
            _f16_shape.clear()
        v = _f16_shape[key] = bool(_lib.lib().regtr_gemm_x3_f16_supported(M, N, K, 1 if with_stats else 0))
    return v


class _GemmTimer:
    __slots__ = ('rec', 'e0', 'meta')

    def __init__(self, rec, **meta):
        self.rec, self.meta = rec, meta
        if rec is not None:
            self.e0 = torch.cuda.Event(enable_timing=True)
            self.e0.record()

    def done(self, **more):
        if self.rec is not None:
            e1 = torch.cuda.Event(enable_timing=True)
            e1.record()
            self.rec.append((self.e0, e1, dict(self.meta, **more)))


_x3_shape = {}


def _x3_plan(M, N, K):
    p = _x3_shape.get((M, N, K))
    if p is None:
        L = _lib.lib()
        ok = bool(L.regtr_gemm_x3_supported(M, N, K))
        p = (ok, bool(ok and L.regtr_gemm_x3_preferred(M, N, K)), L.regtr_gemm_x3_ws_bytes(M, N, K) if ok else 0,
             (L.regtr_gemm_x3_stat_tile_rows(M, N, K) if M > 0 else 0) if ok else 0, L.regtr_gemm_x3_tile_rows(M, N, K) if ok else 0)
        if len(_x3_shape) > 4096:
            _x3_shape.clear()
        _x3_shape[(M, N, K)] = p
    return p


def gemm(a, b, bias=None, row_div=None, residual=None, relu=False, out=None, a_stats=None, a_seg_off=None, a_slope=0.1,
         want_stats=None, eps=1e-5, planes=3):
    L = _lib.lib()
    M, K = a.shape
    sw = b if isinstance(b, SplitWeight) else None
    b_kn = sw.kn if sw is not None else b
    Kb, N = b_kn.shape
    assert K == Kb and a.stride(1) == 1 and b_kn.is_contiguous()
    if (sw is not None and sw.planes is not None and want_stats is not None and bias is None and row_div is None and residual is None
            and not relu and planes == 3 and out is None and stream_ok(M, N, K, a, a_stats)
            and (a_stats is None or a_seg_off is want_stats[0])):
        tm = _GemmTimer(context.current().gemm_records, M=M, N=N, K=K, route='one-shot strip (bf16x3)', terms=6, w_bytes=6, fold=a_stats is not None, stats=True)
        res = gemm_stream(a, sw, want_stats[0], a_stats=a_stats, a_slope=a_slope, want_stats=True, eps=eps)
        tm.done()
        return res
    if out is None:
        out = torch.empty((M, N), dtype=torch.float32, device=a.device)
    ldr = residual.stride(0) if residual is not None else 0
    lda = a.stride(0) if M > 1 else K
    ldc = out.stride(0) if M > 1 else N
    n_seg = a_seg_off.numel() - 1 if a_stats is not None else 0
    x3_ok, x3_pref, nb, x3_R, x3_rows = _x3_plan(M, N, K) if sw is not None and sw.planes is not None else (False, False, 0, 0, 0)
    ctx = context.current()
    use_f16_pair = ctx.f16_pair and not ctx.force_x3
    if ctx.force_x3:
        planes = 3
    f16_range_log = ctx.f16_range_log
    if (x3_ok and lda % 4 == 0 and a.data_ptr() % 16 == 0 and not force_f32_gemm and (N >= 64 or a_stats is None)
            and (force_x3_gemm or x3_pref)):
        ws = _ws(nb, a.device) if nb else None
        R = x3_R if want_stats is not None else 0
        partial, s_off, n_clouds = None, None, 0
        if R:
            s_off = want_stats[0]
            n_clouds = s_off.numel() - 1
            partial = torch.empty((((M + R - 1) // R + n_clouds) * N, 2), dtype=torch.float64, device=a.device)
        seg_rows = s_off if R else a_seg_off
        ti = None
        if seg_rows is not None and (a_seg_off is None or s_off is None or a_seg_off is s_off):
            ti = tile_segments(seg_rows, M, x3_rows)
        pl, npl = sw.planes, int(planes)
        if use_f16_pair and npl >= 2 and sw.f16_ok and f16_pair_ok(M, N, K, R > 0 or a_stats is not None or ti is not None):
            pl, npl = sw.planes16, 4
            if f16_range_log is not None:
                f16_range_log.append((M, N, K, float(a.abs().max()) if M else 0.0, float(sw.kn.abs().max())))
        tm = _GemmTimer(ctx.gemm_records, M=M, N=N, K=K, route='split GEMM (f16 pair)' if npl == 4 else f'split GEMM (bf16 x{npl})',
                        terms={4: 3, 3: 6, 2: 3, 1: 1}[npl], w_bytes={4: 4, 3: 6, 2: 4, 1: 2}[npl], fold=a_stats is not None, stats=R > 0)
        check(L.regtr_gemm_x3(raw(a), lda, bptr(pl), raw(out), ldc, M, N, K, ptr(bias), ptr(row_div),
                              raw(residual), ldr, 1 if relu else 0,
                              ptr(a_stats), iptr(a_seg_off), n_seg, a_slope, bptr(ws), nb, dptr(partial), iptr(s_off), n_clouds,
                              npl, iptr(ti), ctx.status_ptr(), stream()), 'regtr_gemm_x3')
        tm.done()
        if R:
            stats = torch.empty((n_clouds, N, 2), dtype=torch.float32, device=a.device)
            check(L.regtr_instnorm_finalize_tiles(dptr(partial), iptr(s_off), n_clouds, N, R, eps, ptr(stats), stream()),
                  'regtr_instnorm_finalize_tiles')
            return out, stats
    else:
        nb = L.regtr_gemm_f32_ws_bytes(M, N, K)
        ws = _ws(nb, a.device) if nb else None
        tm = _GemmTimer(ctx.gemm_records, M=M, N=N, K=K, route='exact-f32 MFMA', terms=0, w_bytes=4, fold=a_stats is not None, stats=False)
        check(L.regtr_gemm_f32(raw(a), lda, ptr(b_kn), N, raw(out), ldc, M, N, K, ptr(bias), ptr(row_div),
                               raw(residual), ldr, 1 if relu else 0,
                               ptr(a_stats), iptr(a_seg_off), n_seg, a_slope, bptr(ws), nb, stream()), 'regtr_gemm_f32')
        tm.done()
    if want_stats is not None:
        return out, instnorm_stats(out, want_stats[0], want_stats[1], eps)
    return out


def tile_segments(seg_off, M, rows):
    cache = getattr(seg_off, '_regtr_tiles', None)
    if cache is None:
        cache = seg_off._regtr_tiles = {}
    key = (M, rows, seg_off.data_ptr(), seg_off._version)
    t = cache.get(key)
    if t is None:
        t = torch.empty(((M + rows - 1) // rows, 4), dtype=torch.int32, device=seg_off.device)
        check(_lib.lib().regtr_tile_segments(iptr(seg_off), seg_off.numel() - 1, M, rows, iptr(t), stream()), 'regtr_tile_segments')
        for k in [k for k in cache if k[2:] != key[2:]]:
            del cache[k]
        cache[key] = t
    return t


def stream_ok(M, N, K, a, a_stats=None):
    return bool(use_stream_gemm and not force_f32_gemm and not force_x3_gemm and M >= STREAM_MIN_ROWS and a.stride(1) == 1
                and a.stride(0) % 4 == 0 and a.data_ptr() % 16 == 0 and (a_stats is None or K <= 64)
                and _lib.lib().regtr_gemm_stream_supported(M, N, K))


def gemm_stream(a, sw, seg_off, a_stats=None, a_slope=0.1, want_stats=False, eps=1e-5):
    L = _lib.lib()
    M, K = a.shape
    N = sw.N
    n_clouds = seg_off.numel() - 1
    R = L.regtr_gemm_stream_tile_rows()
    ti = tile_segments(seg_off, M, R)
    partial = None
    if want_stats:
        partial = torch.empty((((M + R - 1) // R + n_clouds) * N, 2), dtype=torch.float64, device=a.device)
    out = torch.empty((M, N), dtype=torch.float32, device=a.device)
    check(L.regtr_gemm_stream(raw(a), a.stride(0) if M > 1 else K, bptr(sw.planes), ptr(out), N, M, N, K, ptr(a_stats), a_slope,
                              iptr(seg_off), n_clouds, iptr(ti), dptr(partial), stream()), 'regtr_gemm_stream')
    if not want_stats:
        return out
    stats = torch.empty((n_clouds, N, 2), dtype=torch.float32, device=a.device)
    check(L.regtr_instnorm_finalize_tiles(dptr(partial), iptr(seg_off), n_clouds, N, R, eps, ptr(stats), stream()),
          'regtr_instnorm_finalize_tiles')
    return out, stats


def block_tail_ok(x1, x1_stats, f, sw1, sw2):
    M, K1 = x1.shape
    return bool(use_block_tail and not force_f32_gemm and not force_x3_gemm and M >= STREAM_MIN_ROWS and f.shape[0] == M
                and x1_stats is not None and sw1.N == sw2.N and x1.stride(1) == 1 and f.stride(1) == 1
                and x1.stride(0) % 4 == 0 and f.stride(0) % 4 == 0 and x1.data_ptr() % 16 == 0 and f.data_ptr() % 16 == 0
                and x1_stats.data_ptr() % 16 == 0 and _lib.lib().regtr_block_tail_supported(M, sw1.N, K1, f.shape[1]))


def block_tail(x1, x1_stats, f, sw1, sw2, seg_off, max_len, slope=0.1, eps=1e-5, want_stats=False):
    return _block_tail(x1, x1_stats, None, f, sw1.kn, sw2.kn, seg_off, max_len, slope, eps, want_stats)


def _block_tail(x1, x1_stats, row_div, f, w1_kn, w2_kn, seg_off, max_len, slope, eps, want_stats):
    L = _lib.lib()
    M, K1 = x1.shape
    K2, N = (f.shape[1] if f is not None else 0), w1_kn.shape[1]
    n_clouds = seg_off.numel() - 1
    nb = L.regtr_block_tail_ws_bytes(n_clouds, int(max_len), N, K1, K2)
    ws = torch.empty(nb, dtype=torch.uint8, device=x1.device)
    ti = tile_segments(seg_off, M, 256)
    y = torch.empty((M, N), dtype=torch.float32, device=x1.device)
    st = torch.empty((2 if K2 else 1, n_clouds, N, 2), dtype=torch.float32, device=x1.device) if want_stats else None
    tm = _GemmTimer(context.current().gemm_records, M=M, N=N, K=K1 + K2, route='block tail (moments + two-source strip, bf16x3)', terms=6, w_bytes=6,
                    fold=True, stats=True, passes=2)
    check(L.regtr_block_tail(raw(x1), x1.stride(0), ptr(x1_stats), slope, ptr(row_div), raw(f) if f is not None else None,
                             f.stride(0) if f is not None else 0, ptr(w1_kn), ptr(w2_kn), iptr(seg_off), n_clouds, int(max_len),
                             iptr(ti), M, N, K1, K2, eps, slope, ptr(y), N, bptr(ws), nb, ptr(st), stream()), 'regtr_block_tail')
    tm.done()
    return (y, st) if want_stats else y


def first_block_ok(nq, Cin, KP, Cout):
    return bool(use_block_tail and not force_f32_gemm and not force_x3_gemm and Cin == 1 and KP == 15 and nq >= STREAM_MIN_ROWS
                and _lib.lib().regtr_block_tail_supported(nq, Cout, 16, 0))


def kpconv_norm_lrelu(q_xyz, s_xyz, nbr, x, w16_kn, kernel_points, extent, seg_off, max_len, xyzf=None, slope=0.1, eps=1e-5,
                      want_stats=False):
    L = _lib.lib()
    nq, H = nbr.shape
    ns = x.shape[0]
    KP = kernel_points.shape[0]
    wf = torch.empty((nq, 16), dtype=torch.float32, device=x.device)
    num = torch.empty(nq, dtype=torch.float32, device=x.device)
    rec = context.current().gather_records
    if rec is not None:
        e0, e1, e2 = (torch.cuda.Event(enable_timing=True) for _ in range(3))
        e0.record()
    check(L.regtr_kpconv_gather(ptr(q_xyz), nq, ptr(s_xyz), ns, iptr(nbr), H, ptr(x), 1, None, ptr(xyzf), ptr(kernel_points), KP,
                                float(extent), None, None, 0, slope, ptr(wf), 16, ptr(num), stream()), 'regtr_kpconv_gather')
    if rec is not None:
        e1.record()
    res = _block_tail(wf, None, num, None, w16_kn, None, seg_off, max_len, slope, eps, want_stats)
    if rec is not None:
        e2.record()
        rec.append((e0, e1, e2, nq, H, 1, w16_kn.shape[1]))
    return res


STREAM_MIN_ROWS = 131072
SMALL_REGIME_ROWS = 131072
use_stream_gemm = True
use_block_tail = True
PRENORM_MIN_ROWS = 65536
prenorm_gather = True
PREAPPLY_MIN_ROWS = 8192
assert PREAPPLY_MIN_ROWS == 8192, 'csrc/encoder.hip compiles this gate in (ENC_PREAPPLY_ROWS)'
use_one_call_cross_encoder = True
use_one_call_encoder = True
force_f32_gemm = False
force_x3_gemm = False


def layernorm(x, gamma, beta, add=None, eps=1e-5, want_plain=False, out=None):
    n, D = x.shape
    y = torch.empty_like(x) if out is None else out
    yp = torch.empty_like(x) if want_plain else None
    check(_lib.lib().regtr_layernorm(ptr(x), n, D, ptr(gamma), ptr(beta), eps, ptr(add), ptr(y), ptr(yp), stream()),
          'regtr_layernorm')
    return (y, yp) if want_plain else y


def add(a, b):
    assert a.shape == b.shape
    out = torch.empty_like(a)
    check(_lib.lib().regtr_add_f32(ptr(a), ptr(b), a.numel(), ptr(out), stream()), 'regtr_add_f32')
    return out


_posemb_tables = {}


def posemb_sine(xyz, d_model, scale=1.0, temperature=10000):
    n_dim = 3
    npf = d_model // n_dim // 2 * 2
    key = (npf, temperature, float(scale), xyz.device)
    ent = _posemb_tables.get(key)
    if ent is None:
        dim_t = torch.arange(npf, dtype=torch.float32)
        dim_t = (temperature ** (2 * torch.div(dim_t, 2, rounding_mode='trunc') / npf)).to(xyz.device)
        ent = _posemb_tables[key] = (dim_t, torch.tensor(scale * 2 * math.pi, dtype=torch.float32).item())
    dim_t, scale32 = ent
    pe = torch.empty((xyz.shape[0], d_model), dtype=torch.float32, device=xyz.device)
    check(_lib.lib().regtr_posemb_sine(ptr(xyz), xyz.shape[0], npf, d_model, scale32, ptr(dim_t), ptr(pe), stream()),
          'regtr_posemb_sine')
    return pe


def kpconv(q_xyz, s_xyz, nbr, x, w_flat, kernel_points, extent, x_stats=None, s_seg_off=None, q_seg_off=None, slope=0.1,
           want_stats=None, xyzf=None):
    L = _lib.lib()
    assert xyzf is None or x_stats is None
    nq, H = nbr.shape
    ns, Cin = x.shape
    KP = kernel_points.shape[0]
    dev = x.device
    n_seg = s_seg_off.numel() - 1 if x_stats is not None else 0
    fused_flag = (L.regtr_kpconv_gather_computes_flag(Cin, H) and x.data_ptr() % 16 == 0 and ns > 0 and ns * Cin < (1 << 29)
                  and (x_stats is None or x_stats.data_ptr() % 16 == 0))
    flag = None
    if not fused_flag:
        xyzf = None
        flag = torch.empty(ns, dtype=torch.float32, device=dev)
        check(L.regtr_rowsum_positive(ptr(x), ns, Cin, ptr(x_stats), iptr(s_seg_off) if x_stats is not None else None, n_seg,
                                      slope, ptr(flag), stream()), 'regtr_rowsum_positive')
    wf = torch.empty((nq, KP * Cin), dtype=torch.float32, device=dev)
    num = torch.empty(nq, dtype=torch.float32, device=dev)
    rec = context.current().gather_records
    if rec is not None:
        e0, e1, e2 = (torch.cuda.Event(enable_timing=True) for _ in range(3))
        e0.record()
    check(L.regtr_kpconv_gather(ptr(q_xyz), nq, ptr(s_xyz), ns, iptr(nbr), H, ptr(x), Cin, ptr(flag), ptr(xyzf),
                                ptr(kernel_points), KP, float(extent), ptr(x_stats),
                                iptr(q_seg_off) if x_stats is not None else None, n_seg, slope, ptr(wf), 0, ptr(num), stream()),
          'regtr_kpconv_gather')
    if rec is not None:
        e1.record()
    res = gemm(wf, w_flat, row_div=num, want_stats=want_stats)
    if rec is not None:
        e2.record()
        rec.append((e0, e1, e2, nq, H, Cin, (res[0] if want_stats is not None else res).shape[1]))
    return res




def maxpool(x, nbr, width=None):
    ns, C = x.shape
    nq, H = nbr.shape
    out = torch.empty((nq, C), dtype=torch.float32, device=x.device)
    check(_lib.lib().regtr_maxpool_gather(ptr(x), ns, C, iptr(nbr), H, nq, H if width is None else int(width), ptr(out), stream()),
          'regtr_maxpool_gather')
    return out


def instnorm_stats(x, seg_off, max_len, eps=1e-5):
    L = _lib.lib()
    n_clouds = seg_off.numel() - 1
    C = x.shape[1]
    stats = torch.empty((n_clouds, C, 2), dtype=torch.float32, device=x.device)
    nb = L.regtr_instnorm_ws_bytes(n_clouds, max_len, C)
    ws = _ws(nb, x.device)
    check(L.regtr_instnorm_stats(ptr(x), iptr(seg_off), n_clouds, int(max_len), C, eps, ptr(stats), bptr(ws), nb,
                                 stream()), 'regtr_instnorm_stats')
    return stats


def instnorm_apply(x, seg_off, max_len, stats, residual=None, res_stats=None, lrelu=False, slope=0.1, out=None, row_positive=None,
                   row_xyz=None):
    assert row_xyz is None or (row_positive is not None and row_positive.shape == (x.shape[0], 4) and row_xyz.shape == (x.shape[0], 3))
    n_clouds = seg_off.numel() - 1
    C = x.shape[1]
    if out is None:
        out = torch.empty_like(x)
    check(_lib.lib().regtr_instnorm_apply(ptr(x), iptr(seg_off), n_clouds, int(max_len), C, ptr(stats), ptr(residual),
                                          ptr(res_stats), 1 if lrelu else 0, slope, ptr(out), ptr(row_xyz), ptr(row_positive), stream()),
          'regtr_instnorm_apply')
    return out


def mha(q, k, v, seg_off, kv_of, max_len, n_heads, precision=0):
    N, E = q.shape
    hd = E // n_heads
    out = torch.empty((N, E), dtype=torch.float32, device=q.device)
    ctx = context.current()
    rec = ctx.mha_records
    if ctx.force_x3 and precision == 3:
        precision = 0
    if rec is not None:
        e0, e1 = torch.cuda.Event(enable_timing=True), torch.cuda.Event(enable_timing=True)
        e0.record()
    check(_lib.lib().regtr_mha_fwd(raw(q), q.stride(0), raw(k), k.stride(0), raw(v), v.stride(0),
                                   ptr(out), E, iptr(seg_off), iptr(kv_of), seg_off.numel() - 1, int(max_len), n_heads, hd,
                                   1.0 / math.sqrt(hd), int(precision), ctx.status_ptr(), stream()), 'regtr_mha_fwd')
    if rec is not None:
        e1.record()
        rec.append((e0, e1))
    return out


def mha_bwd(q, k, v, d_out, seg_off, kv_of, max_len, n_heads, out=None):
    L = _lib.lib()
    N, E = q.shape
    hd = E // n_heads
    if out is None:
        out = torch.zeros((N, 3 * E), dtype=torch.float32, device=q.device)
    elif tuple(out.shape) != (N, 3 * E):
        raise RuntimeError(f'mha_bwd: out must be ({N}, {3 * E}), got {tuple(out.shape)}')
    for t in (q, k, v, d_out):
        if tuple(t.shape) != (N, E) or (E > 1 and t.stride(1) != 1):
            raise RuntimeError(f'mha_bwd: q, k, v and d_out must be ({N}, {E}) views with unit column stride')
    base = ptr(out)
    nb = L.regtr_mha_bwd_ws_bytes(N, n_heads)
    ws = _ws(max(nb, 1), q.device)
    ld = lambda t: t.stride(0) if N > 1 else E
    check(L.regtr_mha_bwd(raw(q), ld(q), raw(k), ld(k), raw(v), ld(v), raw(d_out), ld(d_out),
                          base, 3 * E, base + 4 * E if base else None, 3 * E, base + 8 * E if base else None, 3 * E,
                          iptr(seg_off), iptr(kv_of), seg_off.numel() - 1, N, int(max_len), n_heads, hd, 1.0 / math.sqrt(hd),
                          bptr(ws), nb, stream()), 'regtr_mha_bwd')
    return out[:, :E], out[:, E:2 * E], out[:, 2 * E:]


def layernorm_bwd(x, gamma, dy, dres=None, eps=1e-5, out=None):
    L = _lib.lib()
    n, D = x.shape
    for name, t in (('dy', dy), ('dres', dres), ('out', out)):
        if t is not None and tuple(t.shape) != (n, D):
            raise RuntimeError(f'layernorm_bwd: {name} must be ({n}, {D}), got {tuple(t.shape)}')
    dx = torch.empty_like(x) if out is None else out
    dgb = torch.zeros((2, D), dtype=torch.float32, device=x.device)
    nb = L.regtr_layernorm_bwd_ws_bytes(n, D)
    ws = _ws(max(nb, 1), x.device)
    base = ptr(dgb)
    check(L.regtr_layernorm_bwd(ptr(x), n, D, ptr(gamma), eps, ptr(dy), ptr(dres), ptr(dx), base, base + 4 * D, bptr(ws), nb, stream()),
          'regtr_layernorm_bwd')
    return dx, dgb[0], dgb[1]


def bias_relu_bwd(g, h=None, inplace=False):
    L = _lib.lib()
    n, N = g.shape
    if N > 1 and g.stride(1) != 1:
        raise RuntimeError('bias_relu_bwd: g must have unit column stride')
    dh = None
    if h is not None:
        if tuple(h.shape) != (n, N) or (N > 1 and h.stride(1) != 1):
            raise RuntimeError(f'bias_relu_bwd: h must be ({n}, {N}) with unit column stride, got {tuple(h.shape)}')
        dh = g if inplace else torch.empty((n, N), dtype=torch.float32, device=g.device)
    db = torch.zeros((N,), dtype=torch.float32, device=g.device)
    nb = L.regtr_bias_relu_bwd_ws_bytes(n, N)
    ws = _ws(max(nb, 1), g.device)
    ld = lambda t: t.stride(0) if n > 1 else N
    check(L.regtr_bias_relu_bwd(raw(g), ld(g), raw(h), ld(h) if h is not None else 0, raw(dh), ld(dh) if dh is not None else 0, ptr(db),
                                n, N, bptr(ws), nb, stream()), 'regtr_bias_relu_bwd')
    return (dh, db) if h is not None else db


def attn_xyz(q, k, xyz, seg_off, kv_of, max_len):
    Lyr, N, D = q.shape
    out = torch.empty((Lyr, N, 3), dtype=torch.float32, device=q.device)
    check(_lib.lib().regtr_attn_xyz(ptr(q), ptr(k), ptr(xyz), ptr(out), iptr(seg_off), iptr(kv_of), seg_off.numel() - 1, N, Lyr,
                                    int(max_len), D, 1.0 / math.sqrt(D), stream()), 'regtr_attn_xyz')
    return out


def weighted_procrustes(kp, corr, logit, seg_off, n_pairs):
    Lyr, N = logit.shape
    pose = torch.empty((Lyr, n_pairs, 3, 4), dtype=torch.float32, device=kp.device)
    check(_lib.lib().regtr_weighted_procrustes(ptr(kp), ptr(corr), ptr(logit), iptr(seg_off), n_pairs, N, Lyr, ptr(pose),
                                               context.current().status_ptr(), stream()), 'regtr_weighted_procrustes')
    return pose


def infonce(anc, pos_t, anc_xyz, pos_xyz, anc_seg_off, pos_seg_off, max_anc, r_p, r_n, anc_pose=None, rows=False):
    L = _lib.lib()
    n_anc, D = anc.shape
    n_pos = pos_t.shape[0]
    B = anc_seg_off.numel() - 1
    dev = anc.device
    out = torch.empty((B, 2), dtype=torch.float32, device=dev)
    rl = torch.empty(n_anc, dtype=torch.float32, device=dev) if rows else None
    rm = torch.empty(n_anc, dtype=torch.float32, device=dev) if rows else None
    nb = L.regtr_infonce_ws_bytes(B, int(max_anc))
    ws = _ws(max(nb, 1), dev)
    lda = anc.stride(0) if n_anc > 1 else D
    ldp = pos_t.stride(0) if n_pos > 1 else D
    assert anc.stride(1) == 1 and pos_t.stride(1) == 1
    check(L.regtr_infonce(raw(anc) if n_anc else None, lda, raw(pos_t) if n_pos else None, ldp, ptr(anc_xyz) if n_anc else None,
                          ptr(pos_xyz) if n_pos else None, iptr(anc_seg_off), iptr(pos_seg_off), B, n_anc, n_pos, int(max_anc), D,
                          float(r_p), float(r_n), ptr(anc_pose), ptr(out), ptr(rl), ptr(rm), bptr(ws), nb, stream()), 'regtr_infonce')
    return (out, rl, rm) if rows else out


def loss_terms(logit, gt_overlap, kp, warped, seg_off, pose):
    B = seg_off.numel() // 2
    N = logit.shape[0]
    pose = pose.contiguous()
    out = torch.empty((B, 5), dtype=torch.float32, device=logit.device)
    check(_lib.lib().regtr_loss_terms(ptr(logit) if N else None, ptr(gt_overlap) if N else None, ptr(kp) if N else None,
                                      ptr(warped) if N else None, iptr(seg_off), B, N, ptr(pose), pose.shape[-2] * pose.shape[-1],
                                      ptr(out), stream()), 'regtr_loss_terms')
    return out


def se3_transform(xyz, seg_off, pose):
    n = xyz.shape[0]
    pose = pose.contiguous()
    out = torch.empty((n, 3), dtype=torch.float32, device=xyz.device)
    check(_lib.lib().regtr_se3_transform(ptr(xyz) if n else None, iptr(seg_off), seg_off.numel() - 1, n, ptr(pose),
                                         pose.shape[-2] * pose.shape[-1], ptr(out) if n else None, stream()), 'regtr_se3_transform')
    return out


def infonce_rows(anc, pos_t, anc_xyz, pos_xyz, anc_seg_off, pos_seg_off, max_anc, r_p, r_n, anc_pose=None):
    L = _lib.lib()
    n_anc, D = anc.shape
    n_pos = pos_t.shape[0]
    B = anc_seg_off.numel() - 1
    dev = anc.device
    out = torch.empty((B, 2), dtype=torch.float32, device=dev)
    lse = torch.empty(n_anc, dtype=torch.float32, device=dev)
    idx = torch.empty(n_anc, dtype=torch.int32, device=dev)
    rm = torch.empty(n_anc, dtype=torch.float32, device=dev)
    nb = L.regtr_infonce_ws_bytes(B, int(max_anc))
    ws = _ws(max(nb, 1), dev)
    lda = anc.stride(0) if n_anc > 1 else D
    ldp = pos_t.stride(0) if n_pos > 1 else D
    assert anc.stride(1) == 1 and pos_t.stride(1) == 1
    check(L.regtr_infonce_rows(raw(anc) if n_anc else None, lda, raw(pos_t) if n_pos else None, ldp, ptr(anc_xyz) if n_anc else None,
                               ptr(pos_xyz) if n_pos else None, iptr(anc_seg_off), iptr(pos_seg_off), B, n_anc, n_pos, int(max_anc), D,
                               float(r_p), float(r_n), ptr(anc_pose), ptr(out), None, ptr(rm) if n_anc else None,
                               ptr(lse) if n_anc else None, iptr(idx) if n_anc else None, bptr(ws), nb, stream()), 'regtr_infonce_rows')
    return out, lse, idx, rm


def infonce_bwd(anc, pos_t, anc_xyz, pos_xyz, anc_seg_off, pos_seg_off, max_anc, max_pos, r_n, saved, grad, mean_div, anc_pose=None):
    out, lse, idx, rm = saved
    n_anc, D = anc.shape
    n_pos = pos_t.shape[0]
    B = anc_seg_off.numel() - 1
    d_anc = torch.empty((n_anc, D), dtype=torch.float32, device=anc.device)
    d_pos = torch.empty((n_pos, D), dtype=torch.float32, device=anc.device)
    check(_lib.lib().regtr_infonce_bwd(ptr(anc) if n_anc else None, D, ptr(pos_t) if n_pos else None, D,
                                       ptr(anc_xyz) if n_anc else None, ptr(pos_xyz) if n_pos else None, iptr(anc_seg_off),
                                       iptr(pos_seg_off), B, n_anc, n_pos, int(max_anc), int(max_pos), D, float(r_n), ptr(anc_pose),
                                       ptr(lse) if n_anc else None, iptr(idx) if n_anc else None, ptr(rm) if n_anc else None, ptr(out),
                                       ptr(grad.reshape(1)), float(mean_div), ptr(d_anc) if n_anc else None, D,
                                       ptr(d_pos) if n_pos else None, D, stream()), 'regtr_infonce_bwd')
    return d_anc, d_pos


def gemm_tn(a, b, fold=False):
    L = _lib.lib()
    M, N1 = a.shape
    N2 = b.shape[1]
    out = torch.empty((N1, N2), dtype=torch.float32, device=a.device)
    nb = L.regtr_gemm_tn_ws_bytes(M, N1, N2)
    ws = _ws(max(nb, 1), a.device)
    check(L.regtr_gemm_tn(ptr(a) if M else None, N1, ptr(b) if M else None, N2, M, N1, N2, int(bool(fold)), ptr(out), N2, bptr(ws), nb,
                          stream()), 'regtr_gemm_tn')
    return out


def corr_l1_bwd(kp, warped, w, seg_off, pose, grad, den):
    n = kp.shape[0]
    pose = pose.contiguous()
    out = torch.empty((n, 3), dtype=torch.float32, device=kp.device)
    check(_lib.lib().regtr_corr_l1_bwd(ptr(kp) if n else None, ptr(warped) if n else None, ptr(w) if n else None, iptr(seg_off),
                                       seg_off.numel() - 1, n, ptr(pose), pose.shape[-2] * pose.shape[-1], ptr(grad.reshape(1)),
                                       ptr(den.reshape(1)), ptr(out) if n else None, stream()), 'regtr_corr_l1_bwd')
    return out


def kpconv_wf(q_xyz, s_xyz, nbr, x, kernel_points, extent):
    L = _lib.lib()
    nq, H = nbr.shape
    ns, Cin = x.shape
    KP = kernel_points.shape[0]
    flag = None
    if not (L.regtr_kpconv_gather_computes_flag(Cin, H) and x.data_ptr() % 16 == 0 and ns > 0 and ns * Cin < (1 << 29)):
        flag = torch.empty(ns, dtype=torch.float32, device=x.device)
        check(L.regtr_rowsum_positive(ptr(x), ns, Cin, None, None, 0, 0.1, ptr(flag), stream()), 'regtr_rowsum_positive')
    wf = torch.empty((nq, KP * Cin), dtype=torch.float32, device=x.device)
    num = torch.empty(nq, dtype=torch.float32, device=x.device)
    check(L.regtr_kpconv_gather(ptr(q_xyz), nq, ptr(s_xyz), ns, iptr(nbr), H, ptr(x), Cin, ptr(flag), None, ptr(kernel_points), KP,
                                float(extent), None, None, 0, 0.1, ptr(wf), 0, ptr(num), stream()), 'regtr_kpconv_gather')
    return wf, num


def nbr_transpose(nbr, ns):
    L = _lib.lib()
    nq, H = nbr.shape
    ns = int(ns)
    row_off = torch.empty(ns + 1, dtype=torch.int32, device=nbr.device)
    entries = torch.empty(max(nq * H, 1), dtype=torch.int32, device=nbr.device)
    nb = L.regtr_nbr_transpose_ws_bytes(nq, H, ns)
    ws = _ws(max(nb, 1), nbr.device)
    check(L.regtr_nbr_transpose(iptr(nbr) if nq else None, nq, H, ns, iptr(row_off), iptr(entries), bptr(ws), nb, stream()),
          'regtr_nbr_transpose')
    return row_off, entries


def kpconv_gather_bwd(dwf, q_xyz, s_xyz, H, kernel_points, extent, transposed, out=None):
    nq, ns, KP = q_xyz.shape[0], s_xyz.shape[0], kernel_points.shape[0]
    if dwf.shape[0] != nq or dwf.shape[1] % KP:
        raise RuntimeError(f'kpconv_gather_bwd: dwf must be ({nq}, {KP} Cin), got {tuple(dwf.shape)}')
    Cin = dwf.shape[1] // KP
    row_off, entries = transposed
    if row_off.numel() != ns + 1 or entries.numel() < nq * H:
        raise RuntimeError(f'kpconv_gather_bwd: the transposed table is not one of a ({nq}, {H}) table over {ns} supports')
    dx = torch.empty((ns, Cin), dtype=torch.float32, device=dwf.device) if out is None else out
    if out is not None and tuple(out.shape) != (ns, Cin):
        raise RuntimeError(f'kpconv_gather_bwd: out must be ({ns}, {Cin}), got {tuple(out.shape)}')
    check(_lib.lib().regtr_kpconv_gather_bwd(ptr(dwf) if nq else None, ptr(q_xyz) if nq else None, nq, ptr(s_xyz), ns, int(H), Cin,
                                             ptr(kernel_points), KP, float(extent), iptr(row_off), iptr(entries), ptr(dx), stream()),
          'regtr_kpconv_gather_bwd')
    return dx


def row_div(x, div):
    n, N = x.shape
    out = torch.empty((n, N), dtype=torch.float32, device=x.device)
    check(_lib.lib().regtr_row_div(ptr(x), N, ptr(div), n, N, ptr(out), N, stream()), 'regtr_row_div')
    return out


def gemm_tn_any(a, b):
    L = _lib.lib()
    M, N1 = a.shape
    N2 = b.shape[1]
    out = torch.empty((N1, N2), dtype=torch.float32, device=a.device)
    nb = L.regtr_gemm_tn_any_ws_bytes(M, N1, N2)
    ws = _ws(max(nb, 1), a.device)
    check(L.regtr_gemm_tn_any(ptr(a) if M else None, N1, ptr(b) if M else None, N2, M, N1, N2, ptr(out), N2, bptr(ws), nb, stream()),
          'regtr_gemm_tn_any')
    return out
```

### regtr_amd/transformer.py

```python
import copy
import ctypes

import torch
import torch.nn as nn

from . import _lib, context, ops
from .kpconv import _prepared, param_fingerprint


class TransformerCrossEncoderLayer(nn.Module):
    def __init__(self, d_model, nhead, dim_feedforward=2048, dropout=0.1, activation='relu', normalize_before=False,
                 sa_val_has_pos_emb=False, ca_val_has_pos_emb=False, attention_type='dot_prod'):
        super().__init__()
        if attention_type != 'dot_prod':
            raise NotImplementedError
        if activation != 'relu':
            raise NotImplementedError('only the ReLU feed-forward of the shipped configs is implemented')
        if dropout != 0.0:
            raise NotImplementedError('dropout must be 0 (as in both shipped configs): neither forward nor forward_grad implements it')
        self.self_attn = nn.MultiheadAttention(d_model, nhead, dropout=dropout)
        self.multihead_attn = nn.MultiheadAttention(d_model, nhead, dropout=dropout)
        self.linear1 = nn.Linear(d_model, dim_feedforward)
        self.linear2 = nn.Linear(dim_feedforward, d_model)
        self.norm1 = nn.LayerNorm(d_model)
        self.norm2 = nn.LayerNorm(d_model)
        self.norm3 = nn.LayerNorm(d_model)
        self.nhead, self.d_model, self.normalize_before = nhead, d_model, normalize_before
        self.sa_val_has_pos_emb, self.ca_val_has_pos_emb = sa_val_has_pos_emb, ca_val_has_pos_emb
        self._cache = {}
        self.gemm_planes, self.attn_precision = 3, 0

    def _wt(self, name, param, rows=None):
        key = name if rows is None else (name, rows)
        return _prepared(self._cache, key, param, lambda w: ops.SplitWeight(w if rows is None else w[rows[0]:rows[1]], 'nk'))

    def _gemm(self, a, w, **kw):
        return ops.gemm(a, w, planes=self.gemm_planes, **kw)

    def _attention(self, attn, tag, x, norm, pe, val_has_pe, seg_off, kv_of, max_len):
        D = self.d_model
        b_in = attn.in_proj_bias.detach()
        if pe is None:
            x2p = ops.layernorm(x, norm.weight.detach(), norm.bias.detach(), eps=norm.eps)
            qkv = self._gemm(x2p, self._wt(tag + '_in', attn.in_proj_weight), bias=b_in)
        elif val_has_pe:
            x2p = ops.layernorm(x, norm.weight.detach(), norm.bias.detach(), add=pe, eps=norm.eps)
            qkv = self._gemm(x2p, self._wt(tag + '_in', attn.in_proj_weight), bias=b_in)
        else:
            x2p, x2 = ops.layernorm(x, norm.weight.detach(), norm.bias.detach(), add=pe, eps=norm.eps, want_plain=True)
            qkv = torch.empty((x.shape[0], 3 * D), dtype=torch.float32, device=x.device)
            b_qk = _prepared(self._cache, tag + '_bqk', attn.in_proj_bias, lambda b: b[:2 * D].contiguous())
            b_v = _prepared(self._cache, tag + '_bv', attn.in_proj_bias, lambda b: b[2 * D:].contiguous())
            self._gemm(x2p, self._wt(tag + '_in', attn.in_proj_weight, (0, 2 * D)), bias=b_qk, out=qkv[:, :2 * D])
            self._gemm(x2, self._wt(tag + '_in', attn.in_proj_weight, (2 * D, 3 * D)), bias=b_v, out=qkv[:, 2 * D:])
        att = ops.mha(qkv[:, :D], qkv[:, D:2 * D], qkv[:, 2 * D:], seg_off, kv_of, max_len, self.nhead, self.attn_precision)
        return self._gemm(att, self._wt(tag + '_out', attn.out_proj.weight), bias=attn.out_proj.bias.detach(), residual=x)

    def _attention_post(self, attn, tag, x, norm, pe, val_has_pe, seg_off, kv_of, max_len):
        D = self.d_model
        b_in = attn.in_proj_bias.detach()
        xp = x if pe is None else ops.add(x, pe)
        if pe is None or val_has_pe:
            qkv = self._gemm(xp, self._wt(tag + '_in', attn.in_proj_weight), bias=b_in)
        else:
            qkv = torch.empty((x.shape[0], 3 * D), dtype=torch.float32, device=x.device)
            b_qk = _prepared(self._cache, tag + '_bqk', attn.in_proj_bias, lambda b: b[:2 * D].contiguous())
            b_v = _prepared(self._cache, tag + '_bv', attn.in_proj_bias, lambda b: b[2 * D:].contiguous())
            self._gemm(xp, self._wt(tag + '_in', attn.in_proj_weight, (0, 2 * D)), bias=b_qk, out=qkv[:, :2 * D])
            self._gemm(x, self._wt(tag + '_in', attn.in_proj_weight, (2 * D, 3 * D)), bias=b_v, out=qkv[:, 2 * D:])
        att = ops.mha(qkv[:, :D], qkv[:, D:2 * D], qkv[:, 2 * D:], seg_off, kv_of, max_len, self.nhead, self.attn_precision)
        y = self._gemm(att, self._wt(tag + '_out', attn.out_proj.weight), bias=attn.out_proj.bias.detach(), residual=x)
        return ops.layernorm(y, norm.weight.detach(), norm.bias.detach(), eps=norm.eps)

    def forward_post(self, x, pe, seg_off, kv_self, kv_cross, max_len):
        x = self._attention_post(self.self_attn, 'sa', x, self.norm1, pe, self.sa_val_has_pos_emb, seg_off, kv_self, max_len)
        x = self._attention_post(self.multihead_attn, 'ca', x, self.norm2, pe, self.ca_val_has_pos_emb, seg_off, kv_cross,
                                 max_len)
        h = self._gemm(x, self._wt('l1', self.linear1.weight), bias=self.linear1.bias.detach(), relu=True)
        y = self._gemm(h, self._wt('l2', self.linear2.weight), bias=self.linear2.bias.detach(), residual=x)
        return ops.layernorm(y, self.norm3.weight.detach(), self.norm3.bias.detach(), eps=self.norm3.eps)

    def forward(self, x, pe, seg_off, kv_self, kv_cross, max_len):
        if not self.normalize_before:
            return self.forward_post(x, pe, seg_off, kv_self, kv_cross, max_len)
        x = self._attention(self.self_attn, 'sa', x, self.norm1, pe, self.sa_val_has_pos_emb, seg_off, kv_self, max_len)
        x = self._attention(self.multihead_attn, 'ca', x, self.norm2, pe, self.ca_val_has_pos_emb, seg_off, kv_cross,
                            max_len)
        x2 = ops.layernorm(x, self.norm3.weight.detach(), self.norm3.bias.detach(), eps=self.norm3.eps)
        h = self._gemm(x2, self._wt('l1', self.linear1.weight), bias=self.linear1.bias.detach(), relu=True)
        return self._gemm(h, self._wt('l2', self.linear2.weight), bias=self.linear2.bias.detach(), residual=x)

    def forward_grad(self, x, pe, seg_off, kv_self, kv_cross, max_len):
        from . import transformer_grad
        return transformer_grad.layer_forward_grad(self, x, pe, seg_off, kv_self, kv_cross, max_len)


class TransformerCrossEncoder(nn.Module):
    def __init__(self, cross_encoder_layer, num_layers, norm=None, return_intermediate=False):
        super().__init__()
        self.layers = nn.ModuleList([copy.deepcopy(cross_encoder_layer) for _ in range(num_layers)])
        self.num_layers, self.norm, self.return_intermediate = num_layers, norm, return_intermediate
        self._table = None

    def forward(self, x, pe, seg_off, kv_self, kv_cross, max_len):
        n_out = self.num_layers if self.return_intermediate else 1
        outs = torch.empty((n_out,) + tuple(x.shape), dtype=torch.float32, device=x.device)
        if self._one_call_ok(x, pe):
            return self._forward_one_call(x, pe, seg_off, kv_self, kv_cross, max_len, outs)
        for li, layer in enumerate(self.layers):
            x = layer(x, pe, seg_off, kv_self, kv_cross, max_len)
            if self.return_intermediate:
                self._final(x, outs[li])
        if not self.return_intermediate:
            self._final(x, outs[0])
        return outs

    def forward_grad(self, x, pe, seg_off, kv_self, kv_cross, max_len):
        from . import transformer_grad
        return transformer_grad.encoder_forward_grad(self, x, pe, seg_off, kv_self, kv_cross, max_len)

    def _one_call_ok(self, x, pe):
        l0 = self.layers[0]
        ctx = context.current()
        if not (ops.use_one_call_cross_encoder and ctx.mha_records is None and ctx.gemm_records is None and ctx.f16_range_log is None
                and not ops.force_f32_gemm and x.dim() == 2 and x.is_contiguous()
                and x.data_ptr() % 16 == 0 and (pe is None or pe.is_contiguous())):
            return False
        for layer in self.layers:
            if not (layer.normalize_before and (pe is None or (layer.sa_val_has_pos_emb and layer.ca_val_has_pos_emb))
                    and layer.gemm_planes == l0.gemm_planes and layer.attn_precision == l0.attn_precision and layer.nhead == l0.nhead
                    and layer.linear1.out_features == l0.linear1.out_features):
                return False
        return bool(_lib.lib().regtr_cross_encoder_supported(x.shape[0], x.shape[1], l0.linear1.out_features, l0.nhead))

    def _f16_pair(self, n):
        l0 = self.layers[0]
        D, F = l0.d_model, l0.linear1.out_features
        ctx = context.current()
        return bool(ctx.f16_pair and not ctx.force_x3 and l0.gemm_planes >= 2 and ops.f16_pair_ok(n, 3 * D, D) and ops.f16_pair_ok(n, D, D)
                    and ops.f16_pair_ok(n, F, D) and ops.f16_pair_ok(n, D, F))

    def _fingerprint(self):
        return param_fingerprint(self)

    def _param_table(self, f16=False):
        fp = self._fingerprint()
        if self._table is None or self._table[0] != fp:
            self._table = (fp, {})
        tables = self._table[1]
        if f16 in tables:
            return tables[f16]
        ptrs, eps = [], []
        if f16:
            for layer in self.layers:
                m = layer._modules
                for tag, w in (('sa_in', m['self_attn'].in_proj_weight), ('sa_out', m['self_attn'].out_proj.weight),
                               ('ca_in', m['multihead_attn'].in_proj_weight), ('ca_out', m['multihead_attn'].out_proj.weight),
                               ('l1', m['linear1'].weight), ('l2', m['linear2'].weight)):
                    if not layer._wt(tag, w).f16_ok:
                        tables[f16] = (None, None)
                        return tables[f16]
        for layer in self.layers:
            m = layer._modules
            sa, ca = m['self_attn'], m['multihead_attn']
            n1, n2, n3, l1, l2 = m['norm1'], m['norm2'], m['norm3'], m['linear1'], m['linear2']
            eps += [n1.eps, n2.eps, n3.eps]
            pl = (lambda sw: sw.planes16) if f16 else (lambda sw: sw.planes)
            for t in (n1.weight, n1.bias, pl(layer._wt('sa_in', sa.in_proj_weight)), sa.in_proj_bias,
                      pl(layer._wt('sa_out', sa.out_proj.weight)), sa.out_proj.bias,
                      n2.weight, n2.bias, pl(layer._wt('ca_in', ca.in_proj_weight)), ca.in_proj_bias,
                      pl(layer._wt('ca_out', ca.out_proj.weight)), ca.out_proj.bias,
                      n3.weight, n3.bias, pl(layer._wt('l1', l1.weight)), l1.bias, pl(layer._wt('l2', l2.weight)), l2.bias):
                ptrs.append(t.data_ptr())
        for layer in self.layers:
            for prm in layer.parameters():
                _lib.ptr(prm.detach())
        tables[f16] = ((ctypes.c_void_p * len(ptrs))(*ptrs), (ctypes.c_float * len(eps))(*eps))
        return tables[f16]

    def _forward_one_call(self, x, pe, seg_off, kv_self, kv_cross, max_len, outs):
        L = _lib.lib()
        l0 = self.layers[0]
        n, D = x.shape
        F = l0.linear1.out_features
        ctx = context.current()
        f16 = self._f16_pair(n)
        planes = 4 if f16 else (3 if ctx.force_x3 else int(l0.gemm_planes))
        attn_precision = 0 if (ctx.force_x3 and l0.attn_precision == 3) else int(l0.attn_precision)
        table, eps = self._param_table(f16)
        if table is None:
            f16, planes = False, (3 if ctx.force_x3 else max(int(l0.gemm_planes), 3 if l0.attn_precision == 3 else 1))
            table, eps = self._param_table(False)
        nb = L.regtr_cross_encoder_ws_bytes(n, D, F)
        ws = torch.empty(nb, dtype=torch.uint8, device=x.device)
        g = b = None
        feps = 0.0
        if self.norm is not None:
            g, b, feps = self.norm.weight.detach(), self.norm.bias.detach(), self.norm.eps
        _lib.check(L.regtr_cross_encoder_fwd(_lib.ptr(x), n, D, F, l0.nhead, self.num_layers, table, eps, _lib.ptr(g), _lib.ptr(b), feps,
                                             1 if self.return_intermediate else 0, _lib.ptr(pe), _lib.iptr(seg_off), _lib.iptr(kv_self),
                                             _lib.iptr(kv_cross), seg_off.numel() - 1, int(max_len), planes,
                                             attn_precision, _lib.bptr(ws), nb, _lib.ptr(outs), ctx.status_ptr(), _lib.stream()),
                   'regtr_cross_encoder_fwd')
        return outs

    def _final(self, x, out):
        if self.norm is None:
            out.copy_(x)
        else:
            ops.layernorm(x, self.norm.weight.detach(), self.norm.bias.detach(), eps=self.norm.eps, out=out)
```

Before: 2219.

## Add LDS-resident attention kernel and fuse final/next-layer layernorms

Adds a resident MHA kernel. One large workgroup (up to 16 waves) per query chunk splits the whole K/V sequence into MFMA operand planes in LDS once, then every wave runs the online-softmax loop from LDS with no double-buffered streaming. It is gated to sequences of 385–512 tokens with enough workgroups, and the shared per-tile math is factored into a helper. Separately, a layernorm2 kernel computes the shared mean and variance once and writes both the final-norm output and the next layer's norm1 (plus pos-emb) input, removing one layernorm pass per intermediate layer in the non-one-call path. The risk is lower occupancy from the large LDS footprint and wasted load work for mostly idle chunks.

Result: slower. 2189 (-1.4%).

```diff
diff --git a/include/regtr_hip.h b/include/regtr_hip.h
--- a/include/regtr_hip.h
+++ b/include/regtr_hip.h
@@ -111,10 +111,15 @@
 int regtr_layernorm(const float* x, int n, int D, const float* gamma, const float* beta, float eps, const float* add,
                     float* y, float* y_plain, void* stream);
 
+int regtr_layernorm2(const float* x, int n, int D, const float* gamma_a, const float* beta_a, float eps_a, float* y_a,
+                     const float* gamma_b, const float* beta_b, float eps_b, const float* add_b, float* y_b, void* stream);
+
 int regtr_posemb_sine(const float* xyz, int n, int npf, int d_model, float scale, const float* dim_t, float* pe,
                       void* stream);
 
 
+#define REGTR_MHA_STREAMING 0x100
+#define REGTR_MHA_RESIDENT  0x200
 int regtr_mha_fwd(const float* q, int ldq, const float* k, int ldk, const float* v, int ldv, float* out, int ldo,
                   const int* seg_off, const int* kv_of, int n_clouds, int max_len, int n_heads, int head_dim, float scale,
                   int precision, int* status, void* stream);
diff --git a/regtr_amd/_lib.py b/regtr_amd/_lib.py
--- a/regtr_amd/_lib.py
+++ b/regtr_amd/_lib.py
@@ -82,6 +82,7 @@
     'regtr_instnorm_finalize_tiles': (_I, [_P, _P, _I, _I, _I, _F, _P, _P]),
     'regtr_add_f32': (_I, [_P, _P, _Z, _P, _P]),
     'regtr_layernorm': (_I, [_P, _I, _I, _P, _P, _F, _P, _P, _P, _P]),
+    'regtr_layernorm2': (_I, [_P, _I, _I, _P, _P, _F, _P, _P, _P, _F, _P, _P, _P]),
     'regtr_posemb_sine': (_I, [_P, _I, _I, _I, _F, _P, _P, _P]),
     'regtr_mha_fwd': (_I, [_P, _I, _P, _I, _P, _I, _P, _I, _P, _P, _I, _I, _I, _I, _F, _I, _P, _P]),
     'regtr_cross_encoder_per_layer_params': (_I, []),
diff --git a/regtr_amd/csrc/attention.hip b/regtr_amd/csrc/attention.hip
--- a/regtr_amd/csrc/attention.hip
+++ b/regtr_amd/csrc/attention.hip
@@ -153,6 +153,11 @@
 #ifndef MHA_WIDE_MIN_WG
 #define MHA_WIDE_MIN_WG 4096
 #endif
+#ifndef MHA_RES_MIN_WG
+#define MHA_RES_MIN_WG 768
+#endif
+#define MHA_RES_MIN_LEN 385
+#define MHA_RES_MAX_LEN 512
 template <int NP, bool F16 = false>
 __device__ __forceinline__ void bf_split8(const float (&x)[8], bf16x8 (&f)[NP])
 {
@@ -193,6 +198,79 @@
 {
     const auto r = __builtin_amdgcn_permlane32_swap(__float_as_uint(x), __float_as_uint(x), false, false);
     return __uint_as_float(r[0]) + __uint_as_float(r[1]);
+}
+
+template <int NP, bool F16, typename Mid>
+__device__ __forceinline__ void mha_tile_math(const unsigned char* ks_tile, const unsigned char* vt_tile, const unsigned (&f_off)[2],
+                                              const bf16x8 (&qf)[2][NP], int kt, int nk, int hi, floatx16& o, floatx16& o_lo,
+                                              float& m_run, float& l_run, Mid&& mid)
+{
+    floatx16 sc, sc_lo;
+#pragma unroll
+    for (int r = 0; r < 16; r++) { sc[r] = 0.f; sc_lo[r] = 0.f; }
+#pragma unroll
+    for (int ks = 0; ks < 2; ks++) {
+        bf16x8 kf[NP];
+#pragma unroll
+        for (int p = 0; p < NP; p++) kf[p] = __builtin_bit_cast(bf16x8, *(const uint4*)(ks_tile + p * (TK * BROW) + f_off[ks]));
+        if constexpr (F16) f16_mma(kf, qf[ks], sc, sc_lo);
+        else sc = bf_mma<NP>(kf, qf[ks], sc);
+    }
+    if constexpr (F16) {
+        rg_fold_low(sc, sc_lo);
+    }
+    mid();
+    if (kt + TK > nk) {
+#pragma unroll
+        for (int r = 0; r < 16; r++)
+            if (kt + acc_row(r, hi) >= nk) sc[r] = -INFINITY;
+    }
+    float mx = -INFINITY;
+#pragma unroll
+    for (int r = 0; r < 16; r++) mx = fmaxf(mx, sc[r]);
+    mx = mha_max_halves(mx);
+    const float m_new = fmaxf(m_run, mx);
+    const float alpha = __builtin_amdgcn_exp2f(m_run - m_new);
+    float pr[16];
+    float psum = 0.f;
+#pragma unroll
+    for (int r = 0; r < 16; r++) { pr[r] = __builtin_amdgcn_exp2f(sc[r] - m_new); psum += pr[r]; }
+    psum = mha_sum_halves(psum);
+    l_run = l_run * alpha + psum;
+    m_run = m_new;
+#pragma unroll
+    for (int r = 0; r < 16; r++) { o[r] *= alpha; if (F16) o_lo[r] *= alpha; }
+#pragma unroll
+    for (int ks = 0; ks < 2; ks++) {
+        float x[8];
+#pragma unroll
+        for (int j = 0; j < 8; j++) x[j] = pr[8 * ks + j];
+        bf16x8 pf[NP], vf[NP];
+        bf_split8<NP, F16>(x, pf);
+#pragma unroll
+        for (int p = 0; p < NP; p++) vf[p] = __builtin_bit_cast(bf16x8, *(const uint4*)(vt_tile + p * (HD * BROW) + f_off[ks]));
+        if constexpr (F16) f16_mma(vf, pf, o, o_lo);
+        else o = bf_mma<NP>(vf, pf, o);
+    }
+}
+
+template <bool F16>
+__device__ __forceinline__ void mha_write_out(const MhaArgs& g, floatx16& o, const floatx16& o_lo, float l_run, const bool& wave_live,
+                                              int qrow, int q_end, int hoff, int hi)
+{
+    if constexpr (F16) {
+        const float chk = fmaf(l_run, 0.f, rg_fold_low(o, o_lo));
+        rg_report_range(g.status, chk, wave_live);
+    }
+    if (wave_live && qrow < q_end) {
+        const float inv = l_run > 0.f ? 1.0f / l_run : 0.f;
+        float* dst = g.out + (size_t)qrow * g.ldo + hoff;
+#pragma unroll
+        for (int r4 = 0; r4 < 4; r4++) {
+            const int d = 8 * r4 + 4 * hi;
+            *(float4*)(dst + d) = make_float4(o[4 * r4] * inv, o[4 * r4 + 1] * inv, o[4 * r4 + 2] * inv, o[4 * r4 + 3] * inv);
+        }
+    }
 }
 
 template <int NP, bool F16 = false, int NW = BW>
@@ -301,53 +379,7 @@
         fetch(rnew, kt + 2 * TK);
         MHA_STAMP(1);
         if (wave_live) {
-            floatx16 sc, sc_lo;
-#pragma unroll
-            for (int r = 0; r < 16; r++) { sc[r] = 0.f; sc_lo[r] = 0.f; }
-#pragma unroll
-            for (int ks = 0; ks < 2; ks++) {
-                bf16x8 kf[NP];
-#pragma unroll
-                for (int p = 0; p < NP; p++) kf[p] = __builtin_bit_cast(bf16x8, *(const uint4*)(&Ks[buf][p][f_off[ks]]));
-                if constexpr (F16) f16_mma(kf, qf[ks], sc, sc_lo);
-                else sc = bf_mma<NP>(kf, qf[ks], sc);
-            }
-            if constexpr (F16) {
-                rg_fold_low(sc, sc_lo);
-            }
-            MHA_STAMP(2);
-            if (kt + TK > nk) {
-#pragma unroll
-                for (int r = 0; r < 16; r++)
-                    if (kt + acc_row(r, hi) >= nk) sc[r] = -INFINITY;
-            }
-            float mx = -INFINITY;
-#pragma unroll
-            for (int r = 0; r < 16; r++) mx = fmaxf(mx, sc[r]);
-            mx = mha_max_halves(mx);
-            const float m_new = fmaxf(m_run, mx);
-            const float alpha = __builtin_amdgcn_exp2f(m_run - m_new);
-            float pr[16];
-            float psum = 0.f;
-#pragma unroll
-            for (int r = 0; r < 16; r++) { pr[r] = __builtin_amdgcn_exp2f(sc[r] - m_new); psum += pr[r]; }
-            psum = mha_sum_halves(psum);
-            l_run = l_run * alpha + psum;
-            m_run = m_new;
-#pragma unroll
-            for (int r = 0; r < 16; r++) { o[r] *= alpha; if (F16) o_lo[r] *= alpha; }
-#pragma unroll
-            for (int ks = 0; ks < 2; ks++) {
-                float x[8];
-#pragma unroll
-                for (int j = 0; j < 8; j++) x[j] = pr[8 * ks + j];
-                bf16x8 pf[NP], vf[NP];
-                bf_split8<NP, F16>(x, pf);
-#pragma unroll
-                for (int p = 0; p < NP; p++) vf[p] = __builtin_bit_cast(bf16x8, *(const uint4*)(&Vt[buf][p][f_off[ks]]));
-                if constexpr (F16) f16_mma(vf, pf, o, o_lo);
-                else o = bf_mma<NP>(vf, pf, o);
-            }
+            mha_tile_math<NP, F16>(&Ks[buf][0][0], &Vt[buf][0][0], f_off, qf, kt, nk, hi, o, o_lo, m_run, l_run, [&] { MHA_STAMP(2); });
             MHA_STAMP(3);
         }
         if (more) stage(rold, buf ^ 1);
@@ -366,20 +398,111 @@
                (int)blockIdx.z, (int)blockIdx.x, wave, (int)wave_live, nk, pt[0], pt[1], pt[2], pt[3], pt[4], pt[5], clock64() - pstart);
 #endif
 
-    if constexpr (F16) {
-        const float chk = fmaf(l_run, 0.f, rg_fold_low(o, o_lo));
-        rg_report_range(g.status, chk, wave_live);
-    }
-    const int qrow = q0 + l31;
-    if (wave_live && qrow < q_end) {
-        const float inv = l_run > 0.f ? 1.0f / l_run : 0.f;
-        float* dst = g.out + (size_t)qrow * g.ldo + hoff;
-#pragma unroll
-        for (int r4 = 0; r4 < 4; r4++) {
-            const int d = 8 * r4 + 4 * hi;
-            *(float4*)(dst + d) = make_float4(o[4 * r4] * inv, o[4 * r4 + 1] * inv, o[4 * r4 + 2] * inv, o[4 * r4 + 3] * inv);
-        }
-    }
+    mha_write_out<F16>(g, o, o_lo, l_run, wave_live, q0 + l31, q_end, hoff, hi);
+}
+
+constexpr int RES_NW = 16;
+constexpr int RES_LDS_BYTES = 160 * 1024;
+template <int NP> constexpr int RES_TILE_B = NP * (TK + HD) * BROW;
+template <int NP> constexpr int RES_MAX_TILES = RES_LDS_BYTES / RES_TILE_B<NP>;
+
+struct MhaResArgs {
+    MhaArgs a;
+    int n_chunks;
+    int n_work;
+    int lds_tiles;
+};
+
+template <int NP, bool F16>
+__global__ void __launch_bounds__(RES_NW * RG_WAVE) k_mha_fwd_res(MhaResArgs ga)
+{
+    extern __shared__ __align__(16) unsigned char res_lds[];
+    const MhaArgs& g = ga.a;
+    const int work = rg_xcd_block(blockIdx.x, gridDim.x);
+    if (work >= ga.n_work) return;
+    const int chunk = work % ga.n_chunks, head = (work / ga.n_chunks) % g.n_heads, cloud = work / (ga.n_chunks * g.n_heads);
+    const int t = threadIdx.x, lane = t & 63, l31 = lane & 31, hi = lane >> 5;
+    const int wave = __builtin_amdgcn_readfirstlane(t >> 6), nwaves = blockDim.x >> 6;
+    const int q_begin = g.seg_off[cloud], q_end = g.seg_off[cloud + 1];
+    if (q_begin + chunk * nwaves * TQ >= q_end) return;
+    const int q0 = q_begin + (chunk * nwaves + wave) * TQ;
+    const bool wave_live = q0 < q_end;
+    const int kc = g.kv_of[cloud];
+    const int k_begin = g.seg_off[kc], nk = min(g.seg_off[kc + 1] - k_begin, ga.lds_tiles * TK);
+    const int hoff = head * HD;
+
+    bf16x8 qf[2][NP];
+    {
+        const int qrow = q0 + l31;
+        const bool live = wave_live && qrow < q_end;
+        const float sc2 = g.scale * 1.44269504088896340736f;
+        const float* qp = g.q + (size_t)(live ? qrow : q_begin) * g.ldq + hoff + 8 * hi;
+        float4 qv[2][2];
+#pragma unroll
+        for (int ks = 0; ks < 2; ks++) { qv[ks][0] = *(const float4*)(qp + 16 * ks); qv[ks][1] = *(const float4*)(qp + 16 * ks + 4); }
+        const float scl = live ? sc2 : 0.f;
+#pragma unroll
+        for (int ks = 0; ks < 2; ks++) {
+            const float x[8] = {qv[ks][0].x * scl, qv[ks][0].y * scl, qv[ks][0].z * scl, qv[ks][0].w * scl,
+                                qv[ks][1].x * scl, qv[ks][1].y * scl, qv[ks][1].z * scl, qv[ks][1].w * scl};
+            bf_split8<NP, F16>(x, qf[ks]);
+        }
+    }
+
+    {
+        constexpr int RES_U = 4;
+        const int n_items = (nk + TK - 1) / TK * 256, nthreads = blockDim.x;
+        const int nk1 = nk > 0 ? nk - 1 : 0;
+        for (int base = t; base < n_items; base += RES_U * nthreads) {
+            float4 kx[RES_U]; float2 v0[RES_U], v1[RES_U];
+#pragma unroll
+            for (int u = 0; u < RES_U; u++) {
+                const int item = base + u * nthreads, kt = (item >> 8) * TK, r = item & 255;
+                const int kr = min(kt + (r >> 3), nk1), va = min(kt + 2 * (r >> 4), nk1), vb = min(kt + 2 * (r >> 4) + 1, nk1);
+                kx[u] = *(const float4*)(g.k + (size_t)(k_begin + kr) * g.ldk + hoff + (r & 7) * 4);
+                v0[u] = *(const float2*)(g.v + (size_t)(k_begin + va) * g.ldv + hoff + (r & 15) * 2);
+                v1[u] = *(const float2*)(g.v + (size_t)(k_begin + vb) * g.ldv + hoff + (r & 15) * 2);
+            }
+#pragma unroll
+            for (int u = 0; u < RES_U; u++) {
+                const int item = base + u * nthreads;
+                if (item >= n_items) break;
+                const unsigned r = item & 255, skey = r >> 3, sdk = (r & 7) * 4, su = r >> 4, sd2 = (r & 15) * 2;
+                unsigned char* tile = res_lds + (size_t)(item >> 8) * RES_TILE_B<NP>;
+                const unsigned k_dst = skey * BROW + (((sdk >> 3) ^ ((skey >> 2) & 3u)) * 16u) + (sdk & 7u) * 2u;
+                const unsigned vpos = ((2u * su) & 0x13u) | (((2u * su) & 4u) << 1) | (((2u * su) & 8u) >> 1);
+                unsigned a[NP], b[NP];
+                rg_split2<NP, F16>(kx[u].x, kx[u].y, a);
+                rg_split2<NP, F16>(kx[u].z, kx[u].w, b);
+#pragma unroll
+                for (int p = 0; p < NP; p++) *(uint2*)(tile + p * (TK * BROW) + k_dst) = make_uint2(a[p], b[p]);
+                rg_split2<NP, F16>(v0[u].x, v1[u].x, a);
+                rg_split2<NP, F16>(v0[u].y, v1[u].y, b);
+#pragma unroll
+                for (int p = 0; p < NP; p++) {
+#pragma unroll
+                    for (int dd = 0; dd < 2; dd++) {
+                        const unsigned row = sd2 + dd;
+                        *(unsigned*)(tile + (NP + p) * (HD * BROW) + row * BROW + (((vpos >> 3) ^ ((row >> 2) & 3u)) * 16u) + (vpos & 7u) * 2u) = dd ? b[p] : a[p];
+                    }
+                }
+            }
+        }
+    }
+    __syncthreads();
+    if (!wave_live) return;
+
+    floatx16 o, o_lo;
+#pragma unroll
+    for (int r = 0; r < 16; r++) { o[r] = 0.f; o_lo[r] = 0.f; }
+    float m_run = -INFINITY, l_run = 0.f;
+    unsigned f_off[2];
+#pragma unroll
+    for (int ks = 0; ks < 2; ks++) f_off[ks] = (unsigned)l31 * BROW + ((((unsigned)(2 * ks + hi)) ^ (((unsigned)l31 >> 2) & 3u)) * 16u);
+    const unsigned char* tile = res_lds;
+    for (int kt = 0; kt < nk; kt += TK, tile += RES_TILE_B<NP>)
+        mha_tile_math<NP, F16>(tile, tile + NP * (TK * BROW), f_off, qf, kt, nk, hi, o, o_lo, m_run, l_run, [] {});
+    mha_write_out<F16>(g, o, o_lo, l_run, wave_live, q0 + l31, q_end, hoff, hi);
 }
 
 struct AttnXyzArgs {
@@ -495,20 +618,42 @@
                   int precision, int* status, void* stream)
 {
     if (!q || !k || !v || !out || !seg_off || !kv_of || n_clouds < 1 || n_heads < 1 || max_len < 0) return RG_ERR_ARG;
-    if (head_dim != HD || precision < 0 || precision > 3) return RG_ERR_ARG;
+    const int route = precision & (REGTR_MHA_STREAMING | REGTR_MHA_RESIDENT);
+    precision &= ~(REGTR_MHA_STREAMING | REGTR_MHA_RESIDENT);
+    if (head_dim != HD || precision < 0 || precision > 3 || route == (REGTR_MHA_STREAMING | REGTR_MHA_RESIDENT)) return RG_ERR_ARG;
     if ((ldq | ldk | ldv | ldo) % 4 || (((uintptr_t)q | (uintptr_t)k | (uintptr_t)v | (uintptr_t)out) % 16)) return RG_ERR_ARG;
     if (max_len == 0) return RG_OK;
     MhaArgs g{q, k, v, out, seg_off, kv_of, ldq, ldk, ldv, ldo, n_heads, scale, status};
     hipStream_t st = (hipStream_t)stream;
     const bool small = (long long)rg_cdiv(max_len, BW * TQ) * n_heads * n_clouds < 512;
-    if (precision == 2 || ((precision == 0 || precision == 3) && small)) {
+    const int res_tiles = rg_cdiv(max_len, TK), res_nw = res_tiles < RES_NW ? res_tiles : RES_NW, res_chunks = rg_cdiv(res_tiles, res_nw);
+    const long long res_wg = (long long)res_chunks * n_heads * n_clouds;
+    const bool res_fits = (precision == 3 && res_tiles <= RES_MAX_TILES<2>) || (precision == 1 && res_tiles <= RES_MAX_TILES<1>);
+    const bool wide = max_len > BW * TQ && (long long)rg_cdiv(max_len, BW8 * TQ) * n_heads * n_clouds >= MHA_WIDE_MIN_WG;
+    const bool resident = res_fits && res_wg < (1 << 30) && route != REGTR_MHA_STREAMING &&
+                          (route == REGTR_MHA_RESIDENT || (!(precision == 3 && small) && !wide && res_wg >= MHA_RES_MIN_WG && max_len >= MHA_RES_MIN_LEN && max_len <= MHA_RES_MAX_LEN));
+    if (resident) {
+        if ((ldv % 2) || ((uintptr_t)v % 8)) return RG_ERR_ARG;
+        const MhaResArgs ga{g, res_chunks, (int)res_wg, res_tiles};
+        const int grid = rg_xcd_grid((int)res_wg);
+        if (precision == 3) {
+            const size_t lds = (size_t)res_tiles * RES_TILE_B<2>;
+            if (!rg_allow_dynamic_lds<k_mha_fwd_res<2, true>>(RES_LDS_BYTES)) return RG_ERR_LAUNCH;
+            k_mha_fwd_res<2, true><<<grid, res_nw * RG_WAVE, lds, st>>>(ga);
+        } else {
+            const size_t lds = (size_t)res_tiles * RES_TILE_B<1>;
+            if (!rg_allow_dynamic_lds<k_mha_fwd_res<1, false>>(RES_LDS_BYTES)) return RG_ERR_LAUNCH;
+            k_mha_fwd_res<1, false><<<grid, res_nw * RG_WAVE, lds, st>>>(ga);
+        }
+    }
+    else if (precision == 2 || ((precision == 0 || precision == 3) && small)) {
         const dim3 grid(rg_cdiv(max_len, TQ), n_heads, n_clouds);
         if ((long long)grid.x * grid.y * grid.z <= 1024 && max_len > 4 * TK) k_mha_fwd<4><<<grid, 4 * RG_WAVE, 0, st>>>(g);
         else k_mha_fwd<1><<<grid, RG_WAVE, 0, st>>>(g);
     }
     else {
         if ((ldv % 2) || ((uintptr_t)v % 8)) return RG_ERR_ARG;
-        if (max_len > BW * TQ && (long long)rg_cdiv(max_len, BW8 * TQ) * n_heads * n_clouds >= MHA_WIDE_MIN_WG) {
+        if (wide) {
             const dim3 grid(rg_cdiv(max_len, BW8 * TQ), n_heads, n_clouds);
             if (precision == 0) k_mha_fwd_bf16<3, false, BW8><<<grid, BW8 * RG_WAVE, 0, st>>>(g);
             else if (precision == 3) k_mha_fwd_bf16<2, true, BW8><<<grid, BW8 * RG_WAVE, 0, st>>>(g);
diff --git a/regtr_amd/csrc/cross_encoder.hip b/regtr_amd/csrc/cross_encoder.hip
--- a/regtr_amd/csrc/cross_encoder.hip
+++ b/regtr_amd/csrc/cross_encoder.hip
@@ -66,8 +66,8 @@
         return regtr_gemm_x3(A, K, W, C, N, M, N, K, (const float*)bias, nullptr, residual, residual ? D : 0, relu, nullptr, nullptr, 0,
                              0.1f, gws, gws_bytes, nullptr, nullptr, 0, gemm_planes, nullptr, status, stream);
     };
-    auto attention = [&](const float* xin, const void* const* P, int g, int in_w, float eps, const int* kv_of, float* xout) {
-        int st = regtr_layernorm(xin, M, D, (const float*)P[g], (const float*)P[g + 1], eps, pe, x2p, nullptr, stream);
+    auto attention = [&](const float* xin, const void* const* P, int g, int in_w, float eps, const int* kv_of, float* xout, bool normed) {
+        int st = normed ? RG_OK : regtr_layernorm(xin, M, D, (const float*)P[g], (const float*)P[g + 1], eps, pe, x2p, nullptr, stream);
         if (st != RG_OK) return st;
         st = gemm(x2p, D, P[in_w], P[in_w + 1], qkv, 3 * D, nullptr, 0);
         if (st != RG_OK) return st;
@@ -78,20 +78,28 @@
     };
 
     const float* cur = x;
+    bool normed = false;
     for (int l = 0; l < n_layers; l++) {
         const void* const* P = layer_params + (size_t)l * CE_PER_LAYER;
         const float* eps = layer_eps + 3 * l;
         float* t1 = (cur == xa) ? xb : xa;
         float* t2 = (t1 == xa) ? xb : xa;
-        CE_TRY(attention(cur, P, CE_N1_G, CE_SA_IN_W, eps[0], kv_self, t1));
-        CE_TRY(attention(t1, P, CE_N2_G, CE_CA_IN_W, eps[1], kv_cross, t2));
+        CE_TRY(attention(cur, P, CE_N1_G, CE_SA_IN_W, eps[0], kv_self, t1, normed));
+        CE_TRY(attention(t1, P, CE_N2_G, CE_CA_IN_W, eps[1], kv_cross, t2, false));
         CE_TRY(regtr_layernorm(t2, M, D, (const float*)P[CE_N3_G], (const float*)P[CE_N3_B], eps[2], nullptr, x2p, nullptr, stream));
         CE_TRY(gemm(x2p, D, P[CE_L1_W], P[CE_L1_B], h, F, nullptr, 1));
         CE_TRY(gemm(h, F, P[CE_L2_W], P[CE_L2_B], t1, D, t2, 0));
         cur = t1;
+        normed = false;
         if (return_intermediate || l == n_layers - 1) {
             float* o = outs + (return_intermediate ? (size_t)l * M * D : 0);
-            if (final_gamma) CE_TRY(regtr_layernorm(cur, M, D, final_gamma, final_beta, final_eps, nullptr, o, nullptr, stream));
+            if (final_gamma && l + 1 < n_layers) {
+                const void* const* Pn = P + CE_PER_LAYER;
+                CE_TRY(regtr_layernorm2(cur, M, D, final_gamma, final_beta, final_eps, o, (const float*)Pn[CE_N1_G], (const float*)Pn[CE_N1_B],
+                                        layer_eps[3 * (l + 1)], pe, x2p, stream));
+                normed = true;
+            }
+            else if (final_gamma) CE_TRY(regtr_layernorm(cur, M, D, final_gamma, final_beta, final_eps, nullptr, o, nullptr, stream));
             else if (hipMemcpyAsync(o, cur, (size_t)M * D * sizeof(float), hipMemcpyDeviceToDevice, (hipStream_t)stream) != hipSuccess)
                 return RG_ERR_LAUNCH;
         }
diff --git a/regtr_amd/csrc/norm.hip b/regtr_amd/csrc/norm.hip
--- a/regtr_amd/csrc/norm.hip
+++ b/regtr_amd/csrc/norm.hip
@@ -225,6 +225,45 @@
     }
 }
 
+__global__ void __launch_bounds__(256) k_layernorm2(const float* __restrict__ x, int n, int D, const float* __restrict__ gamma_a,
+                                                    const float* __restrict__ beta_a, float eps_a, float* __restrict__ y_a,
+                                                    const float* __restrict__ gamma_b, const float* __restrict__ beta_b, float eps_b,
+                                                    const float* __restrict__ add_b, float* __restrict__ y_b)
+{
+    const int row = blockIdx.x * (blockDim.x >> 6) + (threadIdx.x >> 6);
+    if (row >= n) return;
+    const int lane = rg_lane();
+    const float* xr = x + (size_t)row * D;
+    float s = 0.f;
+    for (int c = lane * 4; c < D; c += RG_WAVE * 4) {
+        const float4 v = *(const float4*)(xr + c);
+        s += (v.x + v.y) + (v.z + v.w);
+    }
+    const float mean = rg_wave_sum(s) / (float)D;
+    float ss = 0.f;
+    for (int c = lane * 4; c < D; c += RG_WAVE * 4) {
+        const float4 v = *(const float4*)(xr + c);
+        const float a = v.x - mean, b = v.y - mean, cc = v.z - mean, d = v.w - mean;
+        ss += (a * a + b * b) + (cc * cc + d * d);
+    }
+    const float var = rg_wave_sum(ss) / (float)D;
+    const float rstd_a = 1.0f / sqrtf(var + eps_a), rstd_b = 1.0f / sqrtf(var + eps_b);
+    for (int c = lane * 4; c < D; c += RG_WAVE * 4) {
+        const float4 v = *(const float4*)(xr + c);
+        const float4 ga = *(const float4*)(gamma_a + c), ba = *(const float4*)(beta_a + c);
+        *(float4*)(y_a + (size_t)row * D + c) = make_float4((v.x - mean) * rstd_a * ga.x + ba.x, (v.y - mean) * rstd_a * ga.y + ba.y,
+                                                            (v.z - mean) * rstd_a * ga.z + ba.z, (v.w - mean) * rstd_a * ga.w + ba.w);
+        const float4 gb = *(const float4*)(gamma_b + c), bb = *(const float4*)(beta_b + c);
+        float4 o = make_float4((v.x - mean) * rstd_b * gb.x + bb.x, (v.y - mean) * rstd_b * gb.y + bb.y,
+                               (v.z - mean) * rstd_b * gb.z + bb.z, (v.w - mean) * rstd_b * gb.w + bb.w);
+        if (add_b) {
+            const float4 a = *(const float4*)(add_b + (size_t)row * D + c);
+            o.x += a.x; o.y += a.y; o.z += a.z; o.w += a.w;
+        }
+        *(float4*)(y_b + (size_t)row * D + c) = o;
+    }
+}
+
 __global__ void __launch_bounds__(256) k_posemb_sine(const float* __restrict__ xyz, int n, int npf, int d_model, float scale,
                                                      const float* __restrict__ dim_t, float* __restrict__ pe)
 {
@@ -329,6 +368,16 @@
     return RG_OK;
 }
 
+int regtr_layernorm2(const float* x, int n, int D, const float* gamma_a, const float* beta_a, float eps_a, float* y_a,
+                     const float* gamma_b, const float* beta_b, float eps_b, const float* add_b, float* y_b, void* stream)
+{
+    if (!x || !gamma_a || !beta_a || !y_a || !gamma_b || !beta_b || !y_b || y_a == y_b || n < 0 || D < 4 || D % 4) return RG_ERR_ARG;
+    if (n == 0) return RG_OK;
+    k_layernorm2<<<rg_cdiv(n, 4), 256, 0, (hipStream_t)stream>>>(x, n, D, gamma_a, beta_a, eps_a, y_a, gamma_b, beta_b, eps_b, add_b, y_b);
+    RG_RETURN_IF_LAUNCH_FAILED();
+    return RG_OK;
+}
+
 int regtr_posemb_sine(const float* xyz, int n, int npf, int d_model, float scale, const float* dim_t, float* pe,
                       void* stream)
 {
diff --git a/regtr_amd/ops.py b/regtr_amd/ops.py
--- a/regtr_amd/ops.py
+++ b/regtr_amd/ops.py
@@ -360,6 +360,7 @@
 assert PREAPPLY_MIN_ROWS == 8192, 'csrc/encoder.hip compiles this gate in (ENC_PREAPPLY_ROWS)'
 use_one_call_cross_encoder = True
 use_one_call_encoder = True
+use_resident_mha = True
 force_f32_gemm = False
 force_x3_gemm = False
 
@@ -371,6 +372,15 @@
     check(_lib.lib().regtr_layernorm(ptr(x), n, D, ptr(gamma), ptr(beta), eps, ptr(add), ptr(y), ptr(yp), stream()),
           'regtr_layernorm')
     return (y, yp) if want_plain else y
+
+
+def layernorm2(x, gamma_a, beta_a, eps_a, gamma_b, beta_b, eps_b, add_b=None, out_a=None, out_b=None):
+    n, D = x.shape
+    ya = torch.empty_like(x) if out_a is None else out_a
+    yb = torch.empty_like(x) if out_b is None else out_b
+    check(_lib.lib().regtr_layernorm2(ptr(x), n, D, ptr(gamma_a), ptr(beta_a), eps_a, ptr(ya), ptr(gamma_b), ptr(beta_b), eps_b, ptr(add_b),
+                                      ptr(yb), stream()), 'regtr_layernorm2')
+    return ya, yb
 
 
 def add(a, b):
@@ -471,6 +481,10 @@
     return out
 
 
+def mha_route_flag():
+    return 0x200 if use_resident_mha == 'force' else (0 if use_resident_mha else 0x100)
+
+
 def mha(q, k, v, seg_off, kv_of, max_len, n_heads, precision=0):
     N, E = q.shape
     hd = E // n_heads
@@ -484,7 +498,7 @@
         e0.record()
     check(_lib.lib().regtr_mha_fwd(raw(q), q.stride(0), raw(k), k.stride(0), raw(v), v.stride(0),
                                    ptr(out), E, iptr(seg_off), iptr(kv_of), seg_off.numel() - 1, int(max_len), n_heads, hd,
-                                   1.0 / math.sqrt(hd), int(precision), ctx.status_ptr(), stream()), 'regtr_mha_fwd')
+                                   1.0 / math.sqrt(hd), int(precision) | mha_route_flag(), ctx.status_ptr(), stream()), 'regtr_mha_fwd')
     if rec is not None:
         e1.record()
         rec.append((e0, e1))
diff --git a/regtr_amd/transformer.py b/regtr_amd/transformer.py
--- a/regtr_amd/transformer.py
+++ b/regtr_amd/transformer.py
@@ -37,10 +37,13 @@
     def _gemm(self, a, w, **kw):
         return ops.gemm(a, w, planes=self.gemm_planes, **kw)
 
-    def _attention(self, attn, tag, x, norm, pe, val_has_pe, seg_off, kv_of, max_len):
+    def _attention(self, attn, tag, x, norm, pe, val_has_pe, seg_off, kv_of, max_len, x2p=None):
         D = self.d_model
         b_in = attn.in_proj_bias.detach()
-        if pe is None:
+        if x2p is not None:
+            assert pe is None or val_has_pe
+            qkv = self._gemm(x2p, self._wt(tag + '_in', attn.in_proj_weight), bias=b_in)
+        elif pe is None:
             x2p = ops.layernorm(x, norm.weight.detach(), norm.bias.detach(), eps=norm.eps)
             qkv = self._gemm(x2p, self._wt(tag + '_in', attn.in_proj_weight), bias=b_in)
         elif val_has_pe:
@@ -80,10 +83,10 @@
         y = self._gemm(h, self._wt('l2', self.linear2.weight), bias=self.linear2.bias.detach(), residual=x)
         return ops.layernorm(y, self.norm3.weight.detach(), self.norm3.bias.detach(), eps=self.norm3.eps)
 
-    def forward(self, x, pe, seg_off, kv_self, kv_cross, max_len):
+    def forward(self, x, pe, seg_off, kv_self, kv_cross, max_len, x2p=None):
         if not self.normalize_before:
             return self.forward_post(x, pe, seg_off, kv_self, kv_cross, max_len)
-        x = self._attention(self.self_attn, 'sa', x, self.norm1, pe, self.sa_val_has_pos_emb, seg_off, kv_self, max_len)
+        x = self._attention(self.self_attn, 'sa', x, self.norm1, pe, self.sa_val_has_pos_emb, seg_off, kv_self, max_len, x2p=x2p)
         x = self._attention(self.multihead_attn, 'ca', x, self.norm2, pe, self.ca_val_has_pos_emb, seg_off, kv_cross,
                             max_len)
         x2 = ops.layernorm(x, self.norm3.weight.detach(), self.norm3.bias.detach(), eps=self.norm3.eps)
@@ -107,10 +110,17 @@
         outs = torch.empty((n_out,) + tuple(x.shape), dtype=torch.float32, device=x.device)
         if self._one_call_ok(x, pe):
             return self._forward_one_call(x, pe, seg_off, kv_self, kv_cross, max_len, outs)
+        x2p = None
         for li, layer in enumerate(self.layers):
-            x = layer(x, pe, seg_off, kv_self, kv_cross, max_len)
+            x = layer(x, pe, seg_off, kv_self, kv_cross, max_len, x2p=x2p)
+            x2p = None
             if self.return_intermediate:
-                self._final(x, outs[li])
+                nxt = self.layers[li + 1] if li + 1 < len(self.layers) else None
+                if self.norm is not None and nxt is not None and nxt.normalize_before and (pe is None or nxt.sa_val_has_pos_emb):
+                    x2p = ops.layernorm2(x, self.norm.weight.detach(), self.norm.bias.detach(), self.norm.eps, nxt.norm1.weight.detach(),
+                                         nxt.norm1.bias.detach(), nxt.norm1.eps, add_b=pe, out_a=outs[li])[1]
+                else:
+                    self._final(x, outs[li])
         if not self.return_intermediate:
             self._final(x, outs[0])
         return outs
@@ -200,7 +210,7 @@
         _lib.check(L.regtr_cross_encoder_fwd(_lib.ptr(x), n, D, F, l0.nhead, self.num_layers, table, eps, _lib.ptr(g), _lib.ptr(b), feps,
                                              1 if self.return_intermediate else 0, _lib.ptr(pe), _lib.iptr(seg_off), _lib.iptr(kv_self),
                                              _lib.iptr(kv_cross), seg_off.numel() - 1, int(max_len), planes,
-                                             attn_precision, _lib.bptr(ws), nb, _lib.ptr(outs), ctx.status_ptr(), _lib.stream()),
+                                             attn_precision | ops.mha_route_flag(), _lib.bptr(ws), nb, _lib.ptr(outs), ctx.status_ptr(), _lib.stream()),
                    'regtr_cross_encoder_fwd')
         return outs
 
```
